# zzuiekongning/MGDT-YOLO

Hardware: AMD Instinct MI355X
Metric: images/sec @640x640 bs=32 per GPU, detection forward + NMS (whole job: 1 GPU(s)) (higher is better)
Workload: dtype bf16; 1 GPU; mspa_c2f_gd_yolov8-n (MSPA-C2f + GD neck + Detect, nc=80) 640x640 inference, batch 32/GPU: forward + decode + NMS(conf 0.25, iou 0.7), hipGraph replay, 4 batches in flight (one captured graph per resident batch, replayed round-robin on 4 streams); global_batch=32, parallelism=replicas x1 (batch-sharded, no data-path collective), rccl_ranks=1, input=bfloat16 NCHW images, 8 different batches resident in HBM (600 MiB) cycled, detections_last_step=9600, weights=seeded random init (no checkpoints offline), batches_in_flight=4

## Files before the change

include/mgdt.h:

```cpp
#ifndef MGDT_H
#define MGDT_H
#include <stddef.h>
#include <stdint.h>

#ifdef __cplusplus
extern "C" {
#endif

typedef void* mgdt_stream;

typedef enum { MGDT_OK = 0, MGDT_BAD_SHAPE = -1, MGDT_BAD_DTYPE = -2, MGDT_LAUNCH_FAIL = -3, MGDT_BAD_ARG = -4,
               MGDT_WORKSPACE = -5 } mgdt_status;
typedef enum { MGDT_F32 = 0, MGDT_BF16 = 1, MGDT_U8 = 2  } mgdt_dtype;
typedef enum { MGDT_ACT_NONE = 0, MGDT_ACT_SILU = 1, MGDT_ACT_RELU = 2, MGDT_ACT_GELU = 3 } mgdt_act;

typedef struct {
  void* p;
  int32_t n, h, w, c;
  int64_t sn, sh, sw, sc;
} mgdt_view;

const char* mgdt_last_error(void);
const char* mgdt_version(void);

size_t mgdt_conv_packed_bytes(int cin, int cout, int k, int dtype);
int mgdt_conv_pack(const float* w_oihw, const float* conv_bias, const float* bn_gamma, const float* bn_beta,
                   const float* bn_mean, const float* bn_var, float bn_eps, int cin, int cout, int k, int dtype,
                   void* packed_out, float* bias_out, mgdt_stream s);
int mgdt_conv_pack_dgrad(const float* w_oihw, int cin, int cout, int k, int phase, int dtype, void* packed_out, float* bias_out, mgdt_stream s);
typedef struct mgdt_pack_desc {
  const float* w; const float* conv_bias; const float* bn_gamma; const float* bn_beta; const float* bn_mean; const float* bn_var;
  float bn_eps; int32_t cin, cout, k, dtype, mode;
  void* packed; float* bias_out;
} mgdt_pack_desc;
int mgdt_conv_pack_batch(const mgdt_pack_desc* descs, int n, mgdt_stream s);

int mgdt_conv2d_fwd(const mgdt_view* x, const mgdt_view* x2, const float* in_scale, const float* in_shift,
                    const void* packed_w, const float* bias, int k, int stride, int act, const mgdt_view* r1,
                    const mgdt_view* r2, const mgdt_view* y, int dtype, mgdt_stream s);
size_t mgdt_conv_packed_bytes_fp8(int cin, int cout, int k);
int mgdt_conv_pack_fp8(const float* w_oihw, const float* conv_bias, const float* bn_gamma, const float* bn_beta, const float* bn_mean,
                       const float* bn_var, float bn_eps, int cin, int cout, int k, float x_qscale, void* packed_out, float* bias_out,
                       float* oscale_out, mgdt_stream s);
int mgdt_conv2d_fp8_fwd(const mgdt_view* x, const mgdt_view* x2, const float* in_scale, const float* in_shift, const void* packed_w,
                        const float* bias, const float* oscale, float x_qscale, int k, int stride, int act, const mgdt_view* r1,
                        const mgdt_view* r2, const mgdt_view* y, mgdt_stream s);
int mgdt_conv2d_phase_fwd(const mgdt_view* x, const void* packed_w, const float* bias, int phase, const mgdt_view* r1, const mgdt_view* r2,
                          const mgdt_view* y, int dtype, mgdt_stream s);

size_t mgdt_cnx_mlp_packed_bytes(int c, int dtype);
int mgdt_cnx_mlp_pack(const float* w1, const float* b1, const float* w2, const float* b2, int c, void* packed, int dtype, mgdt_stream s);
size_t mgdt_cnx_mlp_workspace_bytes(int n, int h, int w, int c);
int mgdt_cnx_mlp_fwd(const mgdt_view* t, const mgdt_view* res, const void* packed, const float* gamma, const float* beta, void* ws,
                     const mgdt_view* y, int dtype, mgdt_stream s);

int mgdt_cnx_block_supported(int n, int h, int w, int c, int dtype);
size_t mgdt_cnx_block_workspace_bytes(int n, int h, int w, int c);
int mgdt_cnx_block_fwd(const mgdt_view* x, const float* dw_w49c, const float* dw_b, const float* ln_w, const float* ln_b, float eps, const void* packed,
                       const float* gamma, const float* beta, const void* tail_w, const float* tail_b, int tail_act, void* ws, size_t ws_bytes,
                       const mgdt_view* y, int dtype, mgdt_stream s);

size_t mgdt_stem2_packed_bytes(void);
int mgdt_stem2_pack(const float* w_folded, void* packed, mgdt_stream s);
int mgdt_stem2_fwd(const mgdt_view* x, int x_dtype, const void* packed0, const float* bias0, const void* packed1, const float* bias1,
                   const mgdt_view* y, mgdt_stream s);
int mgdt_stem2_geometry(int n, int h, int w, int cu_count, int* out);

int mgdt_detect_tail_supported(int c2, int c3, int nc, int reg_max, int dtype);
int mgdt_detect_tail_fwd(const mgdt_view* tb, const mgdt_view* tc, const void* wb, const float* bb, const void* wc, const float* bc, int nc,
                         float stride, int a_off, int a_total, const mgdt_view* feat, float* y, unsigned long long* best_keys,
                         const void* wb3, const float* bb3, mgdt_stream s);
int mgdt_detect_tail_aug_fwd(const mgdt_view* tb, const mgdt_view* tc, const void* wb, const float* bb, const void* wc, const float* bc, int nc,
                             float stride, int a_off, int a_total, const mgdt_view* feat, float* y, unsigned long long* best_keys,
                             const void* wb3, const float* bb3, float aug_scale, int aug_flip, float aug_img_w, mgdt_stream s);

int mgdt_scale_img_fwd(const mgdt_view* x, int x_dtype, int flip, int hs, int ws, float pad, const mgdt_view* y, int y_dtype, mgdt_stream s);

int mgdt_csp_block_supported(int mode, int cin, int cout, int wd, int nbtl, int h, int w, int dtype);
int mgdt_csp_block_tiles(int mode, int n, int cin, int cout, int wd, int nbtl, int h, int w, int* geom8);
int mgdt_csp_block_fwd(int mode, const mgdt_view* x, const void* front, const float* front_bias, const void* const* mid,
                       const float* const* mid_bias, int nbtl, int shortcut, const void* back, const float* back_bias, int wd, int act,
                       const mgdt_view* y, float* pool, int dtype, mgdt_stream s);

size_t mgdt_pw_chain_packed_bytes(int wd, int dtype);
int mgdt_pw_chain_pack(int idx, const float* w_oi, const float* conv_bias, const float* bn_gamma, const float* bn_beta, const float* bn_mean,
                       const float* bn_var, float bn_eps, int wd, int dtype, void* packed, mgdt_stream s);
int mgdt_pw_chain3_fwd(const mgdt_view* x, const void* packed, int wd, int act, const mgdt_view* y, int dtype, mgdt_stream s);

int mgdt_conv1x1_inject_supported(int cin, int cout, int h, int w, int hg, int wg, int dtype);
int mgdt_conv1x1_inject_fwd(const mgdt_view* x, const void* packed_w, const float* bias, const mgdt_view* ga, const mgdt_view* gf,
                            const mgdt_view* y, int dtype, mgdt_stream s);

int mgdt_conv1x1_inject_conv_supported(int cin, int cmid, int cout2, int h, int w, int hg, int wg, int dtype);
int mgdt_conv1x1_inject_conv_fwd(const mgdt_view* x, const void* packed_w, const float* bias, const mgdt_view* ga, const mgdt_view* gf,
                                 const mgdt_view* gsrc, const void* packed_wg, const float* bias_g, int cmid,
                                 const void* packed_w2, const float* bias2, int act2, const mgdt_view* y2, int dtype, mgdt_stream s);

size_t mgdt_groupnorm_workspace_bytes(int n, int c);
int mgdt_groupnorm_fwd(const mgdt_view* x, const float* gamma, const float* beta, int groups, float eps, int act, void* ws, const mgdt_view* y,
                       int dtype, mgdt_stream s);
int mgdt_tood_layer_attn_fwd(const float* sums, int n, int c, int hw, const float* w1, const float* b1, const float* w2, const float* b2, int hid,
                             int stacked, float* scale, mgdt_stream s);
int mgdt_dcnv2_fwd(const mgdt_view* x, const mgdt_view* offset_mask, const float* w_gemm, const float* bias, const mgdt_view* y, int dtype,
                   mgdt_stream s);
int mgdt_dcnv2_mfma_fwd(const mgdt_view* x, const mgdt_view* offset_mask, const void* packed_w, const mgdt_view* y, int dtype, mgdt_stream s);
int mgdt_pixel_gate_fwd(const mgdt_view* x, const mgdt_view* gate, const mgdt_view* y, int dtype, mgdt_stream s);

int mgdt_conv_pack_direct(const float* w_oihw, const float* conv_bias, const float* bn_gamma, const float* bn_beta,
                          const float* bn_mean, const float* bn_var, float bn_eps, int cin_g, int cout, int k,
                          float* w_out, float* bias_out, mgdt_stream s);
int mgdt_conv2d_direct_fwd(const mgdt_view* x, int x_dtype, const float* w_gemm, const float* bias, int k, int stride,
                           int groups, int act, const mgdt_view* y, int dtype, mgdt_stream s);

#define MGDT_SPR_SPLITS 16
int mgdt_spr_pool_fwd(const mgdt_view* x, float* pooled, int dtype, mgdt_stream s);
int mgdt_spr_attn_fwd(const float* pooled, const float* fc1_w, const float* fc1_b, const float* fc2_w,
                      const float* fc2_b, int n, int c, int groups, int h, int w, int softmax, float* attn, mgdt_stream s);
int mgdt_scale_channels_fwd(const mgdt_view* x, const float* attn, const mgdt_view* y, int dtype, mgdt_stream s);
int mgdt_spr_attn_scale_fwd(const float* pooled, int nsplit, int tiles_x, int tiles_y, const float* fc1_w, const float* fc1_b, const float* fc2_w, const float* fc2_b, int groups,
                            const mgdt_view* x, const mgdt_view* y, const mgdt_view* pool_a, const mgdt_view* pool_b, int dtype, mgdt_stream s);

int mgdt_sppf_pool_fwd(const mgdt_view* x, const mgdt_view* y1, const mgdt_view* y2, const mgdt_view* y3, int dtype,
                       mgdt_stream s);

int mgdt_adaptive_avgpool_fwd(const mgdt_view* x, const mgdt_view* y, int dtype, mgdt_stream s);
int mgdt_bilinear_fwd(const mgdt_view* x, const mgdt_view* y, int dtype, mgdt_stream s);
int mgdt_nearest_fwd(const mgdt_view* x, const mgdt_view* y, int dtype, mgdt_stream s);
int mgdt_copy_fwd(const mgdt_view* x, int x_dtype, const mgdt_view* y, int y_dtype, mgdt_stream s);
int mgdt_image_pad4_fwd(const mgdt_view* x, int x_dtype, const mgdt_view* y, int y_dtype, mgdt_stream s);

#define MGDT_GRN_SPLITS 8
int mgdt_dwconv7_ln_fwd(const mgdt_view* x, const float* dw_w, const float* dw_b, const float* ln_w, const float* ln_b,
                        float eps, const mgdt_view* y, int dtype, mgdt_stream s);
int mgdt_grn_stats_fwd(const mgdt_view* t, const float* gamma, float* ws, float* scale, int dtype, mgdt_stream s);

int mgdt_inject_fwd(const mgdt_view* local, const mgdt_view* ga, const mgdt_view* gf, const mgdt_view* y, int dtype,
                    mgdt_stream s);

int mgdt_detect_decode_fwd(const mgdt_view* feat, int reg_max, int nc, float stride, int a_off, int a_total, float* y,
                           int dtype, mgdt_stream s);
int mgdt_detect_decode_aug_fwd(const mgdt_view* feat, int reg_max, int nc, float stride, int a_off, int a_total, float* y,
                               unsigned long long* best_keys, float aug_scale, int aug_flip, float aug_img_w, int dtype, mgdt_stream s);

size_t mgdt_nms_workspace_bytes(int n, int nc, int a, int multi_label, int max_nms);
int mgdt_nms_fwd(const float* pred, int n, int nc, int a, float conf_thres, float iou_thres, const int32_t* classes,
                 int n_classes, int agnostic, int multi_label, int max_det, int max_nms, float max_wh, float* out,
                 int32_t* kept_anchor, int32_t* counts, const unsigned long long* best_keys, void* ws, size_t ws_bytes, mgdt_stream s);

int mgdt_nms_masks_fwd(const float* pred, int n, int nc, int nm, int a, float conf_thres, float iou_thres, const int32_t* classes,
                       int n_classes, int agnostic, int multi_label, int max_det, int max_nms, float max_wh, float* out,
                       int32_t* kept_anchor, int32_t* counts, const unsigned long long* best_keys, void* ws, size_t ws_bytes, mgdt_stream s);

int mgdt_deconv2x2_fwd(const mgdt_view* x, const void* const* packed4, const float* bias, const mgdt_view* y, int dtype, mgdt_stream s);
int mgdt_seg_concat_fwd(const float* y, int n, int rows, int a_total, const mgdt_view* const* mc, int n_levels, int nm, float* out, int dtype,
                        mgdt_stream s);
int mgdt_seg_mask_geometry(int win_h, int win_w, int out_h, int out_w, int* geom4);
int mgdt_seg_masks_fwd(const mgdt_view* protos, const float* rows, const int32_t* counts, const int32_t* offsets, int max_det, int nm,
                       int top, int left, int win_h, int win_w, int out_h, int out_w, int crop_before, float box_sx, float box_sy,
                       int crop_after, int no_skip, void* out, int out_u8, int dtype, mgdt_stream s);

int mgdt_val_match_fwd(const float* det, const int32_t* ndet, int n, int max_det, const float* labels, const int32_t* nlab, int max_lab,
                       const float* iouv, int n_iou, uint8_t* correct, mgdt_stream s);

size_t mgdt_detect_loss_workspace_bytes(int b, int a_total, int n_gt);
int mgdt_detect_loss_fwd(const mgdt_view* const* feats, const float* strides, int n_levels, int reg_max, int nc,
                         const float* gt, int n_gt, int call_count, float gain_box, float gain_cls, float gain_dfl,
                         float* out5, unsigned char* fg_out, int32_t* gt_idx_out, float* tscore_out, void* ws,
                         size_t ws_bytes, int dtype, mgdt_stream s);
int mgdt_detect_loss_fwd_dev(const mgdt_view* const* feats, const float* strides, int n_levels, int reg_max, int nc,
                             const float* gt, int n_gt, const int32_t* call_count_dev, float gain_box, float gain_cls, float gain_dfl,
                             float* out5, unsigned char* fg_out, int32_t* gt_idx_out, float* tscore_out, void* ws,
                             size_t ws_bytes, int dtype, mgdt_stream s);
int mgdt_detect_loss_bwd(const mgdt_view* const* feats, const mgdt_view* const* grads, const float* strides, int n_levels,
                         int reg_max, int nc, const float* gt, int n_gt, float gain_box, float gain_cls, float gain_dfl,
                         float gscale, const float* out5, void* ws, size_t ws_bytes, int dtype, mgdt_stream s);

size_t mgdt_reduce_workspace_bytes(int c);
int mgdt_bn_stats_fwd(const mgdt_view* y, float eps, float momentum, float* mean, float* rstd, float* running_mean,
                      float* running_var, void* ws, int dtype, mgdt_stream s);
int mgdt_bn_act_fwd(const mgdt_view* y, const float* mean, const float* rstd, const float* gamma, const float* beta, int act,
                    const mgdt_view* r1, const mgdt_view* r2, const mgdt_view* z, int dtype, mgdt_stream s);
int mgdt_bn_act_bwd(const mgdt_view* gz, const mgdt_view* y, const float* mean, const float* rstd, const float* gamma,
                    const float* beta, int act, float* dgamma, float* dbeta, const mgdt_view* dy, void* ws, int dtype, mgdt_stream s);
int mgdt_conv_dgrad(const mgdt_view* dy, const float* w_oihw, int k, int stride, const mgdt_view* dx, int accumulate, int dtype,
                    mgdt_stream s);
int mgdt_gconv_dgrad(const mgdt_view* dy, const float* w, int k, int stride, int groups, const mgdt_view* dx, int accumulate, int dtype,
                     mgdt_stream s);
size_t mgdt_gconv_wgrad_workspace_bytes(int cin, int cout, int k, int groups);
int mgdt_gconv_wgrad(const mgdt_view* x, const mgdt_view* dy, int k, int stride, int groups, float* dw, int accumulate, void* ws, int dtype,
                     mgdt_stream s);
size_t mgdt_conv_wgrad_workspace_bytes(int cin, int cout, int k);
int mgdt_conv_wgrad(const mgdt_view* x, const mgdt_view* x2, const mgdt_view* dy, int k, int stride, float* dw_oihw, float* dbias,
                    int accumulate, void* ws, int dtype, mgdt_stream s);
int mgdt_conv_wgrad_splits(int cin, int cout, int k);
typedef struct mgdt_wgrad_final_desc { const float* partial; float* dw; long n; int32_t nsplit; int32_t accumulate; } mgdt_wgrad_final_desc;
int mgdt_wgrad_final_batch(const mgdt_wgrad_final_desc* descs, int n, mgdt_stream s);
int mgdt_add_fwd(const mgdt_view* a, const mgdt_view* b, const mgdt_view* o, int dtype, mgdt_stream s);
int mgdt_maxpool5_bwd(const mgdt_view* x, const mgdt_view* gy, float* gx_f32, int dtype, mgdt_stream s);
int mgdt_nearest_bwd(const mgdt_view* gy, const mgdt_view* gx, int dtype, mgdt_stream s);

int mgdt_ew_binary(const mgdt_view* a, const mgdt_view* b, const mgdt_view* o, int mode, int dtype, mgdt_stream s);
int mgdt_channel_affine(const mgdt_view* x, const float* scale, const float* shift, const mgdt_view* y, int dtype, mgdt_stream s);
size_t mgdt_nc_reduce_workspace_bytes(int n, int c);
int mgdt_nc_reduce(const mgdt_view* a, const mgdt_view* b, float* out, void* ws, int dtype, mgdt_stream s);
int mgdt_adaptive_avgpool_bwd(const mgdt_view* gy, const mgdt_view* gx, int accumulate, int dtype, mgdt_stream s);
int mgdt_bilinear_bwd(const mgdt_view* gy, const mgdt_view* gx, int accumulate, int dtype, mgdt_stream s);
size_t mgdt_spr_bwd_workspace_bytes(int n, int c, int groups);
int mgdt_spr_bwd(const mgdt_view* gy, const float* pooled_partial, int splits, const float* attn, const float* dattn,
                 const float* fc1_w, const float* fc1_b, const float* fc2_w, const float* fc2_b, int groups,
                 const mgdt_view* gx, float* param_grads, void* ws, int dtype, mgdt_stream s);
int mgdt_dwconv7_ln_train_fwd(const mgdt_view* x, const float* dw_w, const float* dw_b, const float* ln_w, const float* ln_b,
                              float eps, const mgdt_view* y, const mgdt_view* u_out, int dtype, mgdt_stream s);
size_t mgdt_dwconv7_ln_bwd_workspace_bytes(int c);
int mgdt_dwconv7_ln_bwd(const mgdt_view* x, const mgdt_view* u, const mgdt_view* gy, const float* dw_w49c, const float* ln_w, float eps,
                        const mgdt_view* du_tmp, const mgdt_view* dx, int accumulate_dx, float* d_dw_w, float* d_dw_b,
                        float* d_ln_w, float* d_ln_b, void* ws, int dtype, mgdt_stream s);
int mgdt_grn_bwd(const mgdt_view* g, const mgdt_view* t, const float* S, const float* A, const float* B, const float* gamma,
                 const mgdt_view* dt, float* dgamma, float* dbeta, void* ws, int dtype, mgdt_stream s);

size_t mgdt_grad_norm_workspace_bytes(void);
int mgdt_grad_clip_coef(const float* g, long n, float max_norm, float* out2, void* ws, mgdt_stream s);
int mgdt_sgd_step(float* p, const float* g, float* buf, const float* wd, long n, float lr, float lr_bias, float momentum, int nesterov,
                  int first, const float* clip2, mgdt_stream s);
int mgdt_ema_update(float* ema, const float* p, long n, float decay, mgdt_stream s);
int mgdt_sgd_ema_step_dev(float* p, const float* g, float* buf, const float* wd, long n_param, float* ema, long n_total, const float* hyper4,
                          int nesterov, int first, const float* clip2, mgdt_stream s);

int mgdt_box_convert(const float* in, float* out, long n, int row, int mode, mgdt_stream s);
int mgdt_box_iou(const float* b1, int n, const float* b2, int m, float eps, float* out, mgdt_stream s);
int mgdt_bbox_iou(const float* b1, int stride1, const float* b2, int stride2, long n, int xywh, int mode, float eps, float* out, mgdt_stream s);
int mgdt_scale_boxes(float* boxes, long n, int row, float gain, float padx, float pady, float h0, float w0, mgdt_stream s);
int mgdt_letterbox_fwd(const void* src_hwc_bgr, int sh, int sw, long src_pitch, void* dst_chw_rgb, int dh, int dw, int new_h, int new_w, int top,
                       int left, mgdt_stream s);
size_t mgdt_ap_workspace_bytes(int n_det, int n_cls);
int mgdt_ap_per_class(const void* tp, const float* conf, const int32_t* seg, const int32_t* nlab, int n_det, int n_cls, int T, const double* x101,
                      const double* px, double eps, void* ws, double* ap, double* pcur, double* rcur, mgdt_stream s);

int mgdt_gn_affine(const float* Sy, const float* Syy, int n, int c, int hw, const float* gamma, const float* beta, int groups, float eps,
                   float* mean_ng, float* rstd_ng, float* A, float* B, mgdt_stream s);
int mgdt_nc_affine_act_bwd(const mgdt_view* g, const mgdt_view* y, const float* A, const float* B, int act, const mgdt_view* gu, int dtype, mgdt_stream s);
size_t mgdt_gn_bwd_workspace_bytes(int n, int c);
int mgdt_gn_bwd_coef(const float* S1, const float* S2, const float* mean_ng, const float* rstd_ng, const float* gamma, int n, int c, int hw, int groups,
                     float* P, float* Q, float* R, float* dgamma, float* dbeta, int accumulate, void* ws, mgdt_stream s);
int mgdt_nc_axpby(const mgdt_view* a, const float* sa, const mgdt_view* b, const float* sb, const float* shift, const mgdt_view* out, int dtype,
                  mgdt_stream s);
int mgdt_pixel_gate_bwd(const mgdt_view* g, const mgdt_view* x, const mgdt_view* logit, const mgdt_view* gx, const mgdt_view* glogit, int dtype, mgdt_stream s);
size_t mgdt_tood_layer_attn_bwd_workspace_bytes(int n, int c, int hid, int stacked);
int mgdt_tood_layer_attn_bwd(const float* sums, const float* dscale, int n, int c, int hw, const float* w1, const float* b1, const float* w2,
                             const float* b2, int hid, int stacked, float* dsums, float* dw1, float* db1, float* dw2, float* db2, int accumulate,
                             void* ws, mgdt_stream s);
int mgdt_dcn_im2col(const mgdt_view* x, const mgdt_view* om, const mgdt_view* col, int dtype, mgdt_stream s);
int mgdt_dcn_col2im_bwd(const mgdt_view* gcol, const mgdt_view* x, const mgdt_view* om, float* gx_f32, const mgdt_view* gom, int dtype, mgdt_stream s);

#ifdef __cplusplus
}
#endif
#endif
```

mgdt_yolo_amd/_lib.py:

```python
import ctypes as C
import os

_HERE = os.path.dirname(os.path.abspath(__file__))
LIB_PATH = os.environ.get('MGDT_LIB') or os.path.join(_HERE, 'csrc', 'libmgdt_hip.so')

F32, BF16 = 0, 1
ACT_NONE, ACT_SILU, ACT_RELU, ACT_GELU = 0, 1, 2, 3
SPR_SPLITS = 16
GRN_SPLITS = 8


class View(C.Structure):
    _fields_ = [('p', C.c_void_p), ('n', C.c_int32), ('h', C.c_int32), ('w', C.c_int32), ('c', C.c_int32),
                ('sn', C.c_int64), ('sh', C.c_int64), ('sw', C.c_int64), ('sc', C.c_int64)]


VP = C.POINTER(View)
_vp, _i, _f, _sz = C.c_void_p, C.c_int, C.c_float, C.c_size_t

class PackDesc(C.Structure):
    _fields_ = [('w', C.c_void_p), ('conv_bias', C.c_void_p), ('bn_gamma', C.c_void_p), ('bn_beta', C.c_void_p), ('bn_mean', C.c_void_p), ('bn_var', C.c_void_p),
                ('bn_eps', C.c_float), ('cin', C.c_int32), ('cout', C.c_int32), ('k', C.c_int32), ('dtype', C.c_int32), ('mode', C.c_int32),
                ('packed', C.c_void_p), ('bias_out', C.c_void_p)]


class WgradFinalDesc(C.Structure):
    _fields_ = [('partial', C.c_void_p), ('dw', C.c_void_p), ('n', C.c_long), ('nsplit', C.c_int32), ('accumulate', C.c_int32)]


PROTOTYPES = {
    'mgdt_last_error': (C.c_char_p, []),
    'mgdt_version': (C.c_char_p, []),
    'mgdt_conv_packed_bytes': (_sz, [_i, _i, _i, _i]),
    'mgdt_conv_pack': (_i, [_vp, _vp, _vp, _vp, _vp, _vp, _f, _i, _i, _i, _i, _vp, _vp, _vp]),
    'mgdt_conv2d_fwd': (_i, [VP, VP, _vp, _vp, _vp, _vp, _i, _i, _i, VP, VP, VP, _i, _vp]),
    'mgdt_conv_packed_bytes_fp8': (_sz, [_i, _i, _i]),
    'mgdt_conv_pack_fp8': (_i, [_vp, _vp, _vp, _vp, _vp, _vp, _f, _i, _i, _i, _f, _vp, _vp, _vp, _vp]),
    'mgdt_conv2d_fp8_fwd': (_i, [VP, VP, _vp, _vp, _vp, _vp, _vp, _f, _i, _i, _i, VP, VP, VP, _vp]),
    'mgdt_conv_pack_batch': (_i, [_vp, _i, _vp]),
    'mgdt_conv2d_phase_fwd': (_i, [VP, _vp, _vp, _i, VP, VP, VP, _i, _vp]),
    'mgdt_conv_wgrad_splits': (_i, [_i, _i, _i]),
    'mgdt_wgrad_final_batch': (_i, [_vp, _i, _vp]),
    'mgdt_conv_pack_dgrad': (_i, [_vp, _i, _i, _i, _i, _i, _vp, _vp, _vp]),
    'mgdt_conv_pack_direct': (_i, [_vp, _vp, _vp, _vp, _vp, _vp, _f, _i, _i, _i, _vp, _vp, _vp]),
    'mgdt_conv2d_direct_fwd': (_i, [VP, _i, _vp, _vp, _i, _i, _i, _i, VP, _i, _vp]),
    'mgdt_spr_pool_fwd': (_i, [VP, _vp, _i, _vp]),
    'mgdt_spr_attn_fwd': (_i, [_vp, _vp, _vp, _vp, _vp, _i, _i, _i, _i, _i, _i, _vp, _vp]),
    'mgdt_scale_channels_fwd': (_i, [VP, _vp, VP, _i, _vp]),
    'mgdt_sppf_pool_fwd': (_i, [VP, VP, VP, VP, _i, _vp]),
    'mgdt_adaptive_avgpool_fwd': (_i, [VP, VP, _i, _vp]),
    'mgdt_bilinear_fwd': (_i, [VP, VP, _i, _vp]),
    'mgdt_nearest_fwd': (_i, [VP, VP, _i, _vp]),
    'mgdt_copy_fwd': (_i, [VP, _i, VP, _i, _vp]),
    'mgdt_image_pad4_fwd': (_i, [VP, _i, VP, _i, _vp]),
    'mgdt_dwconv7_ln_fwd': (_i, [VP, _vp, _vp, _vp, _vp, _f, VP, _i, _vp]),
    'mgdt_cnx_mlp_packed_bytes': (_sz, [_i, _i]),
    'mgdt_cnx_mlp_pack': (_i, [_vp, _vp, _vp, _vp, _i, _vp, _i, _vp]),
    'mgdt_cnx_mlp_workspace_bytes': (_sz, [_i, _i, _i, _i]),
    'mgdt_cnx_mlp_fwd': (_i, [VP, VP, _vp, _vp, _vp, _vp, VP, _i, _vp]),
    'mgdt_cnx_block_supported': (_i, [_i, _i, _i, _i, _i]),
    'mgdt_cnx_block_workspace_bytes': (_sz, [_i, _i, _i, _i]),
    'mgdt_cnx_block_fwd': (_i, [VP, _vp, _vp, _vp, _vp, _f, _vp, _vp, _vp, _vp, _vp, _i, _vp, _sz, VP, _i, _vp]),
    'mgdt_pw_chain_packed_bytes': (_sz, [_i, _i]),
    'mgdt_pw_chain_pack': (_i, [_i, _vp, _vp, _vp, _vp, _vp, _vp, _f, _i, _i, _vp, _vp]),
    'mgdt_pw_chain3_fwd': (_i, [VP, _vp, _i, _i, VP, _i, _vp]),
    'mgdt_conv1x1_inject_supported': (_i, [_i, _i, _i, _i, _i, _i, _i]),
    'mgdt_conv1x1_inject_fwd': (_i, [VP, _vp, _vp, VP, VP, VP, _i, _vp]),
    'mgdt_conv1x1_inject_conv_supported': (_i, [_i, _i, _i, _i, _i, _i, _i, _i]),
    'mgdt_conv1x1_inject_conv_fwd': (_i, [VP, _vp, _vp, VP, VP, VP, _vp, _vp, _i, _vp, _vp, _i, VP, _i, _vp]),
    'mgdt_spr_attn_scale_fwd': (_i, [_vp, _i, _i, _i, _vp, _vp, _vp, _vp, _i, VP, VP, VP, VP, _i, _vp]),
    'mgdt_stem2_packed_bytes': (_sz, []),
    'mgdt_stem2_pack': (_i, [_vp, _vp, _vp]),
    'mgdt_stem2_fwd': (_i, [VP, _i, _vp, _vp, _vp, _vp, VP, _vp]),
    'mgdt_stem2_geometry': (_i, [_i, _i, _i, _i, C.POINTER(C.c_int)]),
    'mgdt_detect_tail_supported': (_i, [_i, _i, _i, _i, _i]),
    'mgdt_detect_tail_fwd': (_i, [VP, VP, _vp, _vp, _vp, _vp, _i, _f, _i, _i, VP, _vp, _vp, _vp, _vp, _vp]),
    'mgdt_detect_tail_aug_fwd': (_i, [VP, VP, _vp, _vp, _vp, _vp, _i, _f, _i, _i, VP, _vp, _vp, _vp, _vp, _f, _i, _f, _vp]),
    'mgdt_scale_img_fwd': (_i, [VP, _i, _i, _i, _i, _f, VP, _i, _vp]),
    'mgdt_csp_block_supported': (_i, [_i, _i, _i, _i, _i, _i, _i, _i]),
    'mgdt_csp_block_tiles': (_i, [_i, _i, _i, _i, _i, _i, _i, _i, _vp]),
    'mgdt_csp_block_fwd': (_i, [_i, VP, _vp, _vp, _vp, _vp, _i, _i, _vp, _vp, _i, _i, VP, _vp, _i, _vp]),
    'mgdt_groupnorm_workspace_bytes': (_sz, [_i, _i]),
    'mgdt_groupnorm_fwd': (_i, [VP, _vp, _vp, _i, _f, _i, _vp, VP, _i, _vp]),
    'mgdt_tood_layer_attn_fwd': (_i, [_vp, _i, _i, _i, _vp, _vp, _vp, _vp, _i, _i, _vp, _vp]),
    'mgdt_dcnv2_fwd': (_i, [VP, VP, _vp, _vp, VP, _i, _vp]),
    'mgdt_dcnv2_mfma_fwd': (_i, [VP, VP, _vp, VP, _i, _vp]),
    'mgdt_pixel_gate_fwd': (_i, [VP, VP, VP, _i, _vp]),
    'mgdt_gn_affine': (_i, [_vp, _vp, _i, _i, _i, _vp, _vp, _i, _f, _vp, _vp, _vp, _vp, _vp]),
    'mgdt_nc_affine_act_bwd': (_i, [VP, VP, _vp, _vp, _i, VP, _i, _vp]),
    'mgdt_gn_bwd_workspace_bytes': (_sz, [_i, _i]),
    'mgdt_gn_bwd_coef': (_i, [_vp, _vp, _vp, _vp, _vp, _i, _i, _i, _i, _vp, _vp, _vp, _vp, _vp, _i, _vp, _vp]),
    'mgdt_nc_axpby': (_i, [VP, _vp, VP, _vp, _vp, VP, _i, _vp]),
    'mgdt_pixel_gate_bwd': (_i, [VP, VP, VP, VP, VP, _i, _vp]),
    'mgdt_tood_layer_attn_bwd_workspace_bytes': (_sz, [_i, _i, _i, _i]),
    'mgdt_tood_layer_attn_bwd': (_i, [_vp, _vp, _i, _i, _i, _vp, _vp, _vp, _vp, _i, _i, _vp, _vp, _vp, _vp, _vp, _i, _vp, _vp]),
    'mgdt_dcn_im2col': (_i, [VP, VP, VP, _i, _vp]),
    'mgdt_dcn_col2im_bwd': (_i, [VP, VP, VP, _vp, VP, _i, _vp]),
    'mgdt_val_match_fwd': (_i, [_vp, _vp, _i, _i, _vp, _vp, _i, _vp, _i, _vp, _vp]),
    'mgdt_grn_stats_fwd': (_i, [VP, _vp, _vp, _vp, _i, _vp]),
    'mgdt_inject_fwd': (_i, [VP, VP, VP, VP, _i, _vp]),
    'mgdt_detect_decode_fwd': (_i, [VP, _i, _i, _f, _i, _i, _vp, _i, _vp]),
    'mgdt_detect_decode_aug_fwd': (_i, [VP, _i, _i, _f, _i, _i, _vp, _vp, _f, _i, _f, _i, _vp]),
    'mgdt_detect_loss_workspace_bytes': (_sz, [_i, _i, _i]),
    'mgdt_detect_loss_fwd': (_i, [_vp, _vp, _i, _i, _i, _vp, _i, _i, _f, _f, _f, _vp, _vp, _vp, _vp, _vp, _sz, _i, _vp]),
    'mgdt_detect_loss_fwd_dev': (_i, [_vp, _vp, _i, _i, _i, _vp, _i, _vp, _f, _f, _f, _vp, _vp, _vp, _vp, _vp, _sz, _i, _vp]),
    'mgdt_detect_loss_bwd': (_i, [_vp, _vp, _vp, _i, _i, _i, _vp, _i, _f, _f, _f, _f, _vp, _vp, _sz, _i, _vp]),
    'mgdt_reduce_workspace_bytes': (_sz, [_i]),
    'mgdt_bn_stats_fwd': (_i, [VP, _f, _f, _vp, _vp, _vp, _vp, _vp, _i, _vp]),
    'mgdt_bn_act_fwd': (_i, [VP, _vp, _vp, _vp, _vp, _i, VP, VP, VP, _i, _vp]),
    'mgdt_bn_act_bwd': (_i, [VP, VP, _vp, _vp, _vp, _vp, _i, _vp, _vp, VP, _vp, _i, _vp]),
    'mgdt_conv_dgrad': (_i, [VP, _vp, _i, _i, VP, _i, _i, _vp]),
    'mgdt_gconv_dgrad': (_i, [VP, _vp, _i, _i, _i, VP, _i, _i, _vp]),
    'mgdt_gconv_wgrad_workspace_bytes': (_sz, [_i, _i, _i, _i]),
    'mgdt_gconv_wgrad': (_i, [VP, VP, _i, _i, _i, _vp, _i, _vp, _i, _vp]),
    'mgdt_conv_wgrad_workspace_bytes': (_sz, [_i, _i, _i]),
    'mgdt_conv_wgrad': (_i, [VP, VP, VP, _i, _i, _vp, _vp, _i, _vp, _i, _vp]),
    'mgdt_add_fwd': (_i, [VP, VP, VP, _i, _vp]),
    'mgdt_maxpool5_bwd': (_i, [VP, VP, _vp, _i, _vp]),
    'mgdt_nearest_bwd': (_i, [VP, VP, _i, _vp]),
    'mgdt_ew_binary': (_i, [VP, VP, VP, _i, _i, _vp]),
    'mgdt_channel_affine': (_i, [VP, _vp, _vp, VP, _i, _vp]),
    'mgdt_nc_reduce_workspace_bytes': (_sz, [_i, _i]),
    'mgdt_nc_reduce': (_i, [VP, VP, _vp, _vp, _i, _vp]),
    'mgdt_adaptive_avgpool_bwd': (_i, [VP, VP, _i, _i, _vp]),
    'mgdt_bilinear_bwd': (_i, [VP, VP, _i, _i, _vp]),
    'mgdt_spr_bwd_workspace_bytes': (_sz, [_i, _i, _i]),
    'mgdt_spr_bwd': (_i, [VP, _vp, _i, _vp, _vp, _vp, _vp, _vp, _vp, _i, VP, _vp, _vp, _i, _vp]),
    'mgdt_dwconv7_ln_train_fwd': (_i, [VP, _vp, _vp, _vp, _vp, _f, VP, VP, _i, _vp]),
    'mgdt_dwconv7_ln_bwd_workspace_bytes': (_sz, [_i]),
    'mgdt_dwconv7_ln_bwd': (_i, [VP, VP, VP, _vp, _vp, _f, VP, VP, _i, _vp, _vp, _vp, _vp, _vp, _i, _vp]),
    'mgdt_grn_bwd': (_i, [VP, VP, _vp, _vp, _vp, _vp, VP, _vp, _vp, _vp, _i, _vp]),
    'mgdt_grad_norm_workspace_bytes': (_sz, []),
    'mgdt_grad_clip_coef': (_i, [_vp, C.c_long, _f, _vp, _vp, _vp]),
    'mgdt_sgd_step': (_i, [_vp, _vp, _vp, _vp, C.c_long, _f, _f, _f, _i, _i, _vp, _vp]),
    'mgdt_ema_update': (_i, [_vp, _vp, C.c_long, _f, _vp]),
    'mgdt_sgd_ema_step_dev': (_i, [_vp, _vp, _vp, _vp, C.c_long, _vp, C.c_long, _vp, _i, _i, _vp, _vp]),
    'mgdt_box_convert': (_i, [_vp, _vp, C.c_long, _i, _i, _vp]),
    'mgdt_box_iou': (_i, [_vp, _i, _vp, _i, _f, _vp, _vp]),
    'mgdt_bbox_iou': (_i, [_vp, _i, _vp, _i, C.c_long, _i, _i, _f, _vp, _vp]),
    'mgdt_scale_boxes': (_i, [_vp, C.c_long, _i, _f, _f, _f, _f, _f, _vp]),
    'mgdt_letterbox_fwd': (_i, [_vp, _i, _i, C.c_long, _vp, _i, _i, _i, _i, _i, _i, _vp]),
    'mgdt_ap_workspace_bytes': (_sz, [_i, _i]),
    'mgdt_ap_per_class': (_i, [_vp, _vp, _vp, _vp, _i, _i, _i, _vp, _vp, C.c_double, _vp, _vp, _vp, _vp, _vp]),
    'mgdt_nms_workspace_bytes': (_sz, [_i, _i, _i, _i, _i]),
    'mgdt_nms_fwd': (_i, [_vp, _i, _i, _i, _f, _f, _vp, _i, _i, _i, _i, _i, _f, _vp, _vp, _vp, _vp, _vp, _sz, _vp]),
    'mgdt_nms_masks_fwd': (_i, [_vp, _i, _i, _i, _i, _f, _f, _vp, _i, _i, _i, _i, _i, _f, _vp, _vp, _vp, _vp, _vp, _sz, _vp]),
    'mgdt_deconv2x2_fwd': (_i, [VP, _vp, _vp, VP, _i, _vp]),
    'mgdt_seg_concat_fwd': (_i, [_vp, _i, _i, _i, _vp, _i, _i, _vp, _i, _vp]),
    'mgdt_seg_mask_geometry': (_i, [_i, _i, _i, _i, C.POINTER(C.c_int)]),
    'mgdt_seg_masks_fwd': (_i, [VP, _vp, _vp, _vp, _i, _i, _i, _i, _i, _i, _i, _i, _i, _f, _f, _i, _i, _vp, _i, _i, _vp]),
}

_lib = None


def lib():
    global _lib
    if _lib is None:
        if not os.path.exists(LIB_PATH):
            raise RuntimeError(f'{LIB_PATH} is missing: build it with `python -c "import __graft_entry__ as g; g.build()"` '
                               '(mgdt_yolo_amd has no CPU or PyTorch fallback)')
        import torch
        l = C.CDLL(LIB_PATH)
        for name, (res, args) in PROTOTYPES.items():
            fn = getattr(l, name)
            fn.restype, fn.argtypes = res, args
        _lib = l
    return _lib


def check(status, what=''):
    if status != 0:
        raise RuntimeError(f'{what or "mgdt"} failed ({status}): {lib().mgdt_last_error().decode()}')
```

mgdt_yolo_amd/csrc/conv3x3_lds.hip:

```cpp
#include <type_traits>
#include <vector>

#include "common.h"

#define C3_OOB ((int)0x80000000)
#define C3_TW 16
#define C3_RW 18
#define C3_MAXI 14

struct C3Args {
  const char* x; int xsn, xsh, xsw; uint32_t x_bytes;
  char* y; int ysn, ysh, ysw; uint32_t y_bytes;
  const char* wpk; const float* bias;
  int N, H, W, Ho, Wo, Cin, Cout, CP, nchunks, NTtot, ncg, tiles_x, tiles_per_img, ntiles, XP, act;
  FastDiv fd_tpi, fd_tx, fd_cp;
  const float* oscale; float xq;
  unsigned long long* dbg;
};

template <int ACT> __device__ __forceinline__ float c3_act(float v) {
  if (ACT == MGDT_ACT_SILU) return v * fast_sigmoid(v);
  if (ACT == MGDT_ACT_RELU) return fmaxf(v, 0.f);
  return v;
}

template <int NBW, int ACT, int NCH, int MT, bool Q8 = false, int S = 1, int WS = 1>
__global__ __launch_bounds__(256 * WS, 1) void conv3x3_lds_kernel(const C3Args a) {
  constexpr int NTHR = 256 * WS, NBH = (NBW + WS - 1) / WS;
  constexpr int RW = 15 * S + 3, TH = 4 * MT, RH = (TH - 1) * S + 3, RPX = RH * RW;
  constexpr int MAXI = ((S == 1 ? C3_MAXI : 18) + WS - 1) / WS;
  constexpr int WB = Q8 ? 512 : 1024, PB = Q8 ? 8 : 16;
  extern __shared__ __attribute__((aligned(16))) char c3_lds[];
  int* tab = (int*)c3_lds;
  char* wl = c3_lds + (((size_t)a.nchunks * 16 + 15) & ~(size_t)15);
  char* xs = wl + (size_t)a.nchunks * NBW * WB;
  const int tid = threadIdx.x, lane = tid & 63, r = lane & 15, g = lane >> 4;
  const int wave_all = __builtin_amdgcn_readfirstlane(tid >> 6);
  const int wave = wave_all & 3, wcol = wave_all >> 2;
  const int cg = blockIdx.x % a.ncg, w0 = blockIdx.x / a.ncg, wstep = gridDim.x / a.ncg;
  const int nb0 = cg * NBW;
  const __amdgpu_buffer_rsrc_t xrs = __builtin_amdgcn_make_buffer_rsrc((void*)a.x, 0, a.x_bytes, 0x00020000);
  const __amdgpu_buffer_rsrc_t yrs = __builtin_amdgcn_make_buffer_rsrc((void*)a.y, 0, a.y_bytes, 0x00020000);

  for (int p = tid; p < a.nchunks * 4; p += NTHR) {
    const int tap = (int)fdiv((uint32_t)p, a.fd_cp), cp = p - tap * a.CP;
    tab[p] = tap < 9 ? ((tap / 3) * RW + (tap % 3)) * a.XP + cp * PB : 0;
  }
  constexpr int WV = WB / 16;
  {
    const int total = a.nchunks * NBW * WV;
    for (int i0 = tid; i0 < total; i0 += 8 * NTHR) {
      uint4 t[8];
#pragma unroll
      for (int u = 0; u < 8; ++u) {
        const int i = min(i0 + u * NTHR, total - 1);
        const int kc = i / (NBW * WV), rem = i - kc * NBW * WV, bw = rem / WV, ln = rem % WV;
        const bool ok = nb0 + bw < a.NTtot;
        t[u] = ok ? *(const uint4*)(a.wpk + ((size_t)(kc * a.NTtot + nb0 + bw) * WV + ln) * 16) : make_uint4(0u, 0u, 0u, 0u);
      }
#pragma unroll
      for (int u = 0; u < 8; ++u)
        if (i0 + u * NTHR < total) *(uint4*)(wl + (size_t)(i0 + u * NTHR) * 16) = t[u];
    }
  }
  const int nbw0 = nb0 + wcol * NBH;
  f32x4 bias[NBH], osc[Q8 ? NBH : 1];
#pragma unroll
  for (int bw = 0; bw < NBH; ++bw) {
    bias[bw] = nbw0 + bw < a.NTtot ? *(const f32x4*)(a.bias + (nbw0 + bw) * 16 + 4 * g) : f32x4{0.f, 0.f, 0.f, 0.f};
    if constexpr (Q8) {
      osc[bw] = nbw0 + bw < a.NTtot ? *(const f32x4*)(a.oscale + (nbw0 + bw) * 16 + 4 * g) : f32x4{1.f, 1.f, 1.f, 1.f};
      bias[bw] = bias[bw] / osc[bw];
    }
  }

  const int nitems = RPX * a.CP;
  uint4 stage[MAXI];
  auto issue = [&](int t) {
    const int n = (int)fdiv((uint32_t)t, a.fd_tpi), rt = t - n * a.tiles_per_img;
    const int tyi = (int)fdiv((uint32_t)rt, a.fd_tx), txi = rt - tyi * a.tiles_x;
    const int iy0 = tyi * TH * S - 1, ix0 = txi * C3_TW * S - 1;
#pragma unroll
    for (int u = 0; u < MAXI; ++u) {
      const int it = tid + u * NTHR;
      const int pix = (int)fdiv((uint32_t)it, a.fd_cp), c8 = it - pix * a.CP;
      const int py = pix / RW, px = pix - py * RW;
      const int iy = iy0 + py, ix = ix0 + px;
      const bool ok = it < nitems && (unsigned)iy < (unsigned)a.H && (unsigned)ix < (unsigned)a.W;
      stage[u] = __builtin_bit_cast(uint4, __builtin_amdgcn_raw_buffer_load_b128(xrs, ok ? (uint32_t)(n * a.xsn + iy * a.xsh + ix * a.xsw + c8 * 16) : (uint32_t)C3_OOB, 0, 0));
    }
  };
  auto commit = [&]() {
#pragma unroll
    for (int u = 0; u < MAXI; ++u) {
      const int it = tid + u * NTHR;
      if (it < nitems) {
        const int pix = (int)fdiv((uint32_t)it, a.fd_cp), c8 = it - pix * a.CP;
        if constexpr (Q8) *(long*)(xs + pix * a.XP + c8 * 8) = quant8(__builtin_bit_cast(bf16x8, stage[u]), a.xq);
        else *(uint4*)(xs + pix * a.XP + c8 * 16) = stage[u];
      }
    }
  };

  const char* const wlane = wl + lane * PB;
  int bbase[MT];
#pragma unroll
  for (int m = 0; m < MT; ++m) bbase[m] = ((wave * MT + m) * S * RW + r * S) * a.XP;

  __builtin_amdgcn_s_waitcnt(0x0F70);
  unsigned long long T0 = 0, Tc = 0, Tm = 0, Te = 0, tl = 0, ntl = 0;
  if (a.dbg) { T0 = __builtin_amdgcn_s_memrealtime(); tl = T0; }
  int t = w0;
  if (t < a.ntiles) issue(t);
  while (t < a.ntiles) {
    __syncthreads();
    commit();
    __syncthreads();
    if (a.dbg) { const unsigned long long n_ = __builtin_amdgcn_s_memrealtime(); Tc += n_ - tl; tl = n_; }
    const int tn = t + wstep;
    if (tn < a.ntiles) issue(tn);

    f32x4 acc[NBH][MT];
#pragma unroll
    for (int bw = 0; bw < NBH; ++bw)
#pragma unroll
      for (int m = 0; m < MT; ++m) acc[bw][m] = bias[bw];
    typedef typename std::conditional<Q8, long, bf16x8>::type frag_t;
    frag_t A[2][NBH], B[2][MT];
    auto load_frags = [&](int kc, int buf) {
      const int off = tab[kc * 4 + g];
#pragma unroll
      for (int bw = 0; bw < NBH; ++bw) A[buf][bw] = *(const frag_t*)(wlane + (size_t)(kc * NBW + wcol * NBH + bw) * WB);
#pragma unroll
      for (int m = 0; m < MT; ++m) B[buf][m] = *(const frag_t*)(xs + bbase[m] + off);
    };
    auto mm = [&](frag_t w, frag_t p, f32x4 c) __attribute__((always_inline)) {
      if constexpr (Q8) return mma_q8(w, p, c);
      else return __builtin_amdgcn_mfma_f32_16x16x32_bf16(w, p, c, 0, 0, 0);
    };
    load_frags(0, 0);
    if (NCH > 0) {
#pragma unroll
      for (int kc = 0; kc < NCH; ++kc) {
        if (kc + 1 < NCH) load_frags(kc + 1, (kc + 1) & 1);
#pragma unroll
        for (int bw = 0; bw < NBH; ++bw)
#pragma unroll
          for (int m = 0; m < MT; ++m) acc[bw][m] = mm(A[kc & 1][bw], B[kc & 1][m], acc[bw][m]);
      }
    } else {
      for (int kc = 0; kc < a.nchunks; kc += 2) {
        if (kc + 1 < a.nchunks) load_frags(kc + 1, 1);
#pragma unroll
        for (int bw = 0; bw < NBH; ++bw)
#pragma unroll
          for (int m = 0; m < MT; ++m) acc[bw][m] = mm(A[0][bw], B[0][m], acc[bw][m]);
        if (kc + 1 < a.nchunks) {
          if (kc + 2 < a.nchunks) load_frags(kc + 2, 0);
#pragma unroll
          for (int bw = 0; bw < NBH; ++bw)
#pragma unroll
            for (int m = 0; m < MT; ++m) acc[bw][m] = mm(A[1][bw], B[1][m], acc[bw][m]);
        }
      }
    }

    if (a.dbg) { const unsigned long long n_ = __builtin_amdgcn_s_memrealtime(); Tm += n_ - tl; tl = n_; }
    {
      const int n = (int)fdiv((uint32_t)t, a.fd_tpi), rt = t - n * a.tiles_per_img;
      const int tyi = (int)fdiv((uint32_t)rt, a.fd_tx), txi = rt - tyi * a.tiles_x;
#pragma unroll
      for (int m = 0; m < MT; ++m) {
        const int oy = tyi * TH + wave * MT + m, ox = txi * C3_TW + r;
        const bool pin = oy < a.Ho && ox < a.Wo;
        const int po = n * a.ysn + oy * a.ysh + ox * a.ysw;
#pragma unroll
        for (int bw = 0; bw < NBH; ++bw) {
          const int co = (nbw0 + bw) * 16 + 4 * g;
          bf16x4 o;
#pragma unroll
          for (int j = 0; j < 4; ++j) o[j] = (bf16)c3_act<ACT>(Q8 ? acc[bw][m][j] * osc[Q8 ? bw : 0][j] : acc[bw][m][j]);
          __builtin_amdgcn_raw_buffer_store_b64(__builtin_bit_cast(__attribute__((__vector_size__(2 * sizeof(unsigned int)))) unsigned int, o), yrs,
                                                (pin && co < a.Cout) ? (uint32_t)(po + co * 2) : (uint32_t)C3_OOB, 0, 0);
        }
      }
    }
    if (a.dbg) { const unsigned long long n_ = __builtin_amdgcn_s_memrealtime(); Te += n_ - tl; tl = n_; ++ntl; }
    t = tn;
  }
  if (a.dbg && tid == 0) { unsigned long long* d = a.dbg + (size_t)blockIdx.x * 6; d[0] = T0; d[1] = tl; d[2] = Tc; d[3] = Tm; d[4] = Te; d[5] = ntl; }
}

bool mgdt_conv3x3_lds_launch(const mgdt_view* x, const mgdt_view* y, const void* packed_w, const float* bias, int act, int CP, int nchunks, int NTtot, hipStream_t st,
                             const float* q8_oscale, float q8_xq, int stride) {
  const bool q8 = q8_oscale != nullptr;
  static const int mode = getenv("MGDT_CONV3_LDS") ? atoi(getenv("MGDT_CONV3_LDS")) : 1;
  if (!mode) return false;
  static const bool ws2 = !(getenv("MGDT_C3_WAVES8") && atoi(getenv("MGDT_C3_WAVES8")) == 0);
  const bool wide = mode >= 3 || ws2;
  const int Cin = x->c, Cout = y->c;
  if (stride == 2 && (q8_oscale || Cin > 64 || NTtot % 4 || (nchunks != 9 && !(nchunks == 18 && wide)))) return false;
  if (Cin % 8 || Cin < 32 || Cin > 80 || Cout % 4 || Cout < 32 || (act != MGDT_ACT_SILU && act != MGDT_ACT_NONE && act != MGDT_ACT_RELU)) return false;
  const long M = (long)x->n * x->h * x->w;
  if (M < 16 * 1024 || x->h < 16 || x->w < 16) return false;
  const long extx = ((long)(x->n - 1) * x->sn + (long)(x->h - 1) * x->sh + (long)(x->w - 1) * x->sw + x->c) * 2;
  const long exty = ((long)(y->n - 1) * y->sn + (long)(y->h - 1) * y->sh + (long)(y->w - 1) * y->sw + y->c) * 2;
  if (extx >= 0x7fffffffL || exty >= 0x7fffffffL) return false;
  C3Args a;
  memset(&a, 0, sizeof(a));
  a.x = (const char*)x->p; a.xsn = (int)(x->sn * 2); a.xsh = (int)(x->sh * 2); a.xsw = (int)(x->sw * 2); a.x_bytes = (uint32_t)extx;
  a.y = (char*)y->p; a.ysn = (int)(y->sn * 2); a.ysh = (int)(y->sh * 2); a.ysw = (int)(y->sw * 2); a.y_bytes = (uint32_t)exty;
  a.wpk = (const char*)packed_w; a.bias = bias;
  a.N = x->n; a.H = x->h; a.W = x->w; a.Ho = y->h; a.Wo = y->w; a.Cin = Cin; a.Cout = Cout; a.CP = CP; a.nchunks = nchunks; a.NTtot = NTtot; a.act = act;
  a.XP = q8 ? Cin + 16 : Cin * 2 + 16;
  a.oscale = q8_oscale; a.xq = q8_xq;
  const int NBW = stride == 2 ? 4 : NTtot;
  if (NBW != 2 && NBW != 3 && NBW != 4 && NBW != 5 && NBW != 6) return false;
  a.ncg = NTtot / NBW;
  const size_t fixed = (((size_t)nchunks * 16 + 15) & ~(size_t)15) + (size_t)nchunks * NBW * (q8 ? 512 : 1024);
  auto region = [&](int mt) { return stride == 2 ? (size_t)(8 * mt + 1) * 33 * a.XP : (size_t)(4 * mt + 2) * C3_RW * a.XP; };
  int MT = stride == 2 ? 2 : 4;
  if (stride == 1 && fixed + region(MT) > 160 * 1024) MT = NBW == 5 && !q8 && wide && fixed + region(3) <= 160 * 1024 ? 3 : 2;
  const size_t lds = fixed + region(MT);
  if (lds > 160 * 1024) return false;
  if (NBW == 5 && !q8 && MT == 2 && mode < 2) return false;
  if (stride == 1 && (q8 ? MT != 4 : ((NBW == 5 && MT == 4) || (NBW != 5 && MT != 4)))) return false;
  const int TH = 4 * MT;
  a.tiles_x = cdiv(y->w, C3_TW);
  a.tiles_per_img = a.tiles_x * cdiv(y->h, TH);
  a.ntiles = x->n * a.tiles_per_img;
  if ((stride == 2 ? (2 * TH + 1) * 33 * CP > 256 * 18 : (TH + 2) * C3_RW * CP > 256 * C3_MAXI)) return false;
  a.fd_tpi = make_fastdiv((uint32_t)a.tiles_per_img); a.fd_tx = make_fastdiv((uint32_t)a.tiles_x); a.fd_cp = make_fastdiv((uint32_t)CP);
  int nwg = 256 / a.ncg * a.ncg;
  nwg = (int)std::min<long>(nwg, (long)a.ntiles * a.ncg);
  nwg = nwg / a.ncg * a.ncg;
  if (nwg < a.ncg) return false;
 #define C3_LAUNCH_Q8(NB, ACTV)                                                                                      \
  {                                                                                                                  \
    static std::atomic<bool> qattr{false}, qattr18{false}, qattr23{false};                                            \
    if (nchunks == 18) {                                                                                             \
      if (!qattr18) { (void)hipFuncSetAttribute((const void*)conv3x3_lds_kernel<NB, ACTV, 18, 4, true>, hipFuncAttributeMaxDynamicSharedMemorySize, 160 * 1024); qattr18 = true; } \
      conv3x3_lds_kernel<NB, ACTV, 18, 4, true><<<nwg, 256, lds, st>>>(a);                                           \
    } else if (nchunks == 23) {                                                                                      \
      if (!qattr23) { (void)hipFuncSetAttribute((const void*)conv3x3_lds_kernel<NB, ACTV, 23, 4, true>, hipFuncAttributeMaxDynamicSharedMemorySize, 160 * 1024); qattr23 = true; } \
      conv3x3_lds_kernel<NB, ACTV, 23, 4, true><<<nwg, 256, lds, st>>>(a);                                           \
    } else {                                                                                                         \
      if (!qattr) { (void)hipFuncSetAttribute((const void*)conv3x3_lds_kernel<NB, ACTV, 0, 4, true>, hipFuncAttributeMaxDynamicSharedMemorySize, 160 * 1024); qattr = true; } \
      conv3x3_lds_kernel<NB, ACTV, 0, 4, true><<<nwg, 256, lds, st>>>(a);                                            \
    }                                                                                                                \
  }
#define C3_ACT_Q8(NB) \
  if (act == MGDT_ACT_SILU) C3_LAUNCH_Q8(NB, MGDT_ACT_SILU) else if (act == MGDT_ACT_RELU) C3_LAUNCH_Q8(NB, MGDT_ACT_RELU) else C3_LAUNCH_Q8(NB, MGDT_ACT_NONE)
#define C3_LAUNCH(NB, ACTV, MTV, WSV)                                                                                     \
  {                                                                                                                  \
    static std::atomic<bool> attr{false}, attr18{false}, attr23{false};                                                                        \
    if (nchunks == 18) {                                                                                             \
      if (!attr18) { (void)hipFuncSetAttribute((const void*)conv3x3_lds_kernel<NB, ACTV, 18, MTV, false, 1, WSV>, hipFuncAttributeMaxDynamicSharedMemorySize, 160 * 1024); attr18 = true; } \
      conv3x3_lds_kernel<NB, ACTV, 18, MTV, false, 1, WSV><<<nwg, 256 * WSV, lds, st>>>(a);                                                    \
    } else if (nchunks == 23) {                                                                                      \
      if (!attr23) { (void)hipFuncSetAttribute((const void*)conv3x3_lds_kernel<NB, ACTV, 23, MTV, false, 1, WSV>, hipFuncAttributeMaxDynamicSharedMemorySize, 160 * 1024); attr23 = true; } \
      conv3x3_lds_kernel<NB, ACTV, 23, MTV, false, 1, WSV><<<nwg, 256 * WSV, lds, st>>>(a);                                               \
    } else {                                                                                                         \
      if (!attr) { (void)hipFuncSetAttribute((const void*)conv3x3_lds_kernel<NB, ACTV, 0, MTV, false, 1, WSV>, hipFuncAttributeMaxDynamicSharedMemorySize, 160 * 1024); attr = true; } \
      conv3x3_lds_kernel<NB, ACTV, 0, MTV, false, 1, WSV><<<nwg, 256 * WSV, lds, st>>>(a);                                                     \
    }                                                                                                                \
  }
#define C3_ACT(NB, MTV, WSV) \
  if (act == MGDT_ACT_SILU) C3_LAUNCH(NB, MGDT_ACT_SILU, MTV, WSV) else if (act == MGDT_ACT_RELU) C3_LAUNCH(NB, MGDT_ACT_RELU, MTV, WSV) else C3_LAUNCH(NB, MGDT_ACT_NONE, MTV, WSV)
  static unsigned long long* dbgbuf = nullptr;
  if (getenv("MGDT_C3_DBG") && !dbgbuf) (void)hipMalloc((void**)&dbgbuf, 256 * 6 * 8);
  a.dbg = dbgbuf;
#define C3_LAUNCH_S2(ACTV, NCHV)                                                                                      \
  {                                                                                                                  \
    static std::atomic<bool> sattr{false}, sattr8{false};                                                            \
    if (ws2) {                                                                                                       \
      if (!sattr8) { (void)hipFuncSetAttribute((const void*)conv3x3_lds_kernel<4, ACTV, NCHV, 2, false, 2, 2>, hipFuncAttributeMaxDynamicSharedMemorySize, 160 * 1024); sattr8 = true; } \
      conv3x3_lds_kernel<4, ACTV, NCHV, 2, false, 2, 2><<<nwg, 512, lds, st>>>(a);                                   \
    } else {                                                                                                         \
      if (!sattr) { (void)hipFuncSetAttribute((const void*)conv3x3_lds_kernel<4, ACTV, NCHV, 2, false, 2>, hipFuncAttributeMaxDynamicSharedMemorySize, 160 * 1024); sattr = true; } \
      conv3x3_lds_kernel<4, ACTV, NCHV, 2, false, 2><<<nwg, 256, lds, st>>>(a);                                      \
    }                                                                                                                \
  }
#define C3_ACT_S2(NCHV) \
  if (act == MGDT_ACT_SILU) C3_LAUNCH_S2(MGDT_ACT_SILU, NCHV) else if (act == MGDT_ACT_RELU) C3_LAUNCH_S2(MGDT_ACT_RELU, NCHV) else C3_LAUNCH_S2(MGDT_ACT_NONE, NCHV)
  if (stride == 2) {
    if (nchunks == 9) { C3_ACT_S2(9) } else { C3_ACT_S2(18) }
  } else if (q8) {
    if (NBW == 6) { C3_ACT_Q8(6) } else if (NBW == 5) { C3_ACT_Q8(5) } else if (NBW == 4) { C3_ACT_Q8(4) } else if (NBW == 3) { C3_ACT_Q8(3) } else { C3_ACT_Q8(2) }
  } else if (ws2 && (NBW == 6 || NBW == 4 || (NBW == 5 && MT == 3))) {
    if (NBW == 6) { C3_ACT(6, 4, 2) } else if (NBW == 4) { C3_ACT(4, 4, 2) } else { C3_ACT(5, 3, 2) }
  } else if (NBW == 6) { C3_ACT(6, 4, 1) } else if (NBW == 5 && MT == 3) { C3_ACT(5, 3, 1) } else if (NBW == 5) { C3_ACT(5, 2, 1) } else if (NBW == 4) { C3_ACT(4, 4, 1) } else if (NBW == 3) { C3_ACT(3, 4, 1) } else { C3_ACT(2, 4, 1) }
#undef C3_ACT
#undef C3_ACT_Q8
#undef C3_ACT_S2
#undef C3_LAUNCH_S2
#undef C3_LAUNCH_Q8
#undef C3_LAUNCH
  if (dbgbuf) {
    std::vector<unsigned long long> h(256 * 6);
    (void)hipStreamSynchronize(st);
    (void)hipMemcpy(h.data(), dbgbuf, h.size() * 8, hipMemcpyDeviceToHost);
    unsigned long long t0 = ~0ull, t1 = 0; double c = 0, m = 0, e = 0, nt = 0;
    for (int i = 0; i < nwg; ++i) { t0 = std::min(t0, h[i * 6]); t1 = std::max(t1, h[i * 6 + 1]); c += h[i * 6 + 2]; m += h[i * 6 + 3]; e += h[i * 6 + 4]; nt += h[i * 6 + 5]; }
    fprintf(stderr, "conv3x3_lds cin %d cout %d %dx%d: %d wgs, %d tiles, span %.1f us; per tile (us): wait+commit %.2f mfma %.2f epilogue %.2f\n", Cin, Cout, x->h, x->w, nwg,
            a.ntiles, (t1 - t0) * 0.01, c / nt * 0.01, m / nt * 0.01, e / nt * 0.01);
  }
  return true;
}
```

mgdt_yolo_amd/csrc/conv_igemm.hip:

```cpp
#include "conv_igemm_kernel.h"

struct FoldArgs { const float *cb, *g, *b, *mu, *var; float eps; int cout_real, cpad; float* bias_out; };
template <typename T>
__global__ void pack_kernel(const float* __restrict__ w, const float* __restrict__ scale, int Cin, int Cout, int KS,
                            int CP, int nchunks, int NTtot, T* __restrict__ out, int dgrad = 0, FoldArgs fa = FoldArgs{}) {
  constexpr int PE = Piece<T>::PE;
  long total = (long)nchunks * NTtot * 64 * PE;
  if (fa.bias_out && blockIdx.x == 0)
    for (int c = threadIdx.x; c < fa.cpad; c += blockDim.x) {
      float bo = 0.f;
      if (c < fa.cout_real) {
        if (fa.g) {
          const float s = fa.g[c] / sqrtf(fa.eps + fa.var[c]);
          bo = fa.b[c] - fa.g[c] * fa.mu[c] / sqrtf(fa.var[c] + fa.eps);
          if (fa.cb) bo += s * fa.cb[c];
        } else if (fa.cb) {
          bo = fa.cb[c];
        }
      }
      fa.bias_out[c] = bo;
    }
  for (long i = blockIdx.x * (long)blockDim.x + threadIdx.x; i < total; i += (long)gridDim.x * blockDim.x) {
    int j = (int)(i % PE);
    long t = i / PE;
    int lane = (int)(t % 64);
    t /= 64;
    int nb = (int)(t % NTtot);
    int kc = (int)(t / NTtot);
    int r = lane & 15, g = lane >> 4;
    int p = kc * 4 + g;
    int tap = p / CP, cp = p % CP;
    if (dgrad >= 2) {
      const int nc_ = 1 + ((dgrad - 2) & 1), nr_ = 1 + ((dgrad - 2) >> 1);
      tap = tap < nr_ * nc_ ? (1 + tap / nc_) * 3 + (1 + tap % nc_) : 99;
    }
    int cin = cp * PE + j, cout = nb * 16 + r;
    float v = 0.f;
    if (tap < KS * KS && cin < Cin && cout < Cout) {
      if (dgrad == 1) v = w[(((long)cin * Cout + cout) * KS + (KS - 1 - tap / KS)) * KS + (KS - 1 - tap % KS)];
      else if (dgrad >= 2) {
        const int py = (dgrad - 2) >> 1, px = (dgrad - 2) & 1;
        const int ky = py + 1 - 2 * (tap / KS - 1), kx = px + 1 - 2 * (tap % KS - 1);
        v = ((unsigned)ky < 3u && (unsigned)kx < 3u) ? w[(((long)cin * Cout + cout) * 3 + ky) * 3 + kx] : 0.f;
      }
      else v = w[(((long)cout * Cin + cin) * KS + tap / KS) * KS + tap % KS];
      if (scale) v *= scale[cout];
      else if (fa.g) v *= fa.g[cout] / sqrtf(fa.eps + fa.var[cout]);
    }
    out[i] = (T)v;
  }
}

__global__ void fold_kernel(const float* cb, const float* g, const float* b, const float* mu, const float* var, float eps,
                            int Cout, int Cpad, float* scale, float* bias_out) {
  int c = blockIdx.x * blockDim.x + threadIdx.x;
  if (c >= Cpad) return;
  float s = 1.f, bo = 0.f;
  if (c < Cout) {
    if (g) {
      s = g[c] / sqrtf(eps + var[c]);
      bo = b[c] - g[c] * mu[c] / sqrtf(var[c] + eps);
      if (cb) bo += s * cb[c];
    } else if (cb) {
      bo = cb[c];
    }
  }
  scale[c] = s;
  bias_out[c] = bo;
}

static inline int piece_elems(int dtype) { return dtype == MGDT_BF16 ? 8 : 4; }

static inline int phase_ntaps(int mode) { return mode < 2 ? 9 : (1 + ((mode - 2) >> 1)) * (1 + ((mode - 2) & 1)); }
static inline unsigned long long phase_taplist(int mode, int k) {
  unsigned long long l = 0;
  if (mode < 2) { for (int t = 0; t < k * k; ++t) l |= (unsigned long long)t << (4 * t); return l; }
  const int nr = 1 + ((mode - 2) >> 1), nc = 1 + ((mode - 2) & 1);
  for (int i = 0; i < nr * nc; ++i) l |= (unsigned long long)((1 + i / nc) * 3 + (1 + i % nc)) << (4 * i);
  return l;
}
static void conv_geometry(int cin, int cout, int k, int dtype, int* CP, int* nchunks, int* NTtot, int ntaps = 0) {
  int pe = piece_elems(dtype);
  *CP = (cin + pe - 1) / pe;
  int pieces = (ntaps > 0 ? ntaps : k * k) * (*CP);
  *nchunks = (pieces + 3) / 4;
  *NTtot = (cout + 15) / 16;
}

extern "C" size_t mgdt_conv_packed_bytes(int cin, int cout, int k, int dtype) {
  int CP, nchunks, NTtot;
  conv_geometry(cin, cout, k, dtype, &CP, &nchunks, &NTtot);
  return (size_t)nchunks * NTtot * 1024 + (size_t)NTtot * 16 * sizeof(float);
}

extern "C" int mgdt_conv_pack(const float* w, const float* cb, const float* g, const float* b, const float* mu,
                              const float* var, float eps, int cin, int cout, int k, int dtype, void* packed,
                              float* bias_out, mgdt_stream s) {
  if (!w || !packed || !bias_out) MGDT_FAIL(MGDT_BAD_ARG, "conv_pack: null pointer");
  if ((g != nullptr) != (b != nullptr) || (g != nullptr) != (mu != nullptr) || (g != nullptr) != (var != nullptr))
    MGDT_FAIL(MGDT_BAD_ARG, "conv_pack: BN arguments must be all present or all NULL");
  int CP, nchunks, NTtot;
  conv_geometry(cin, cout, k, dtype, &CP, &nchunks, &NTtot);
  hipStream_t st = (hipStream_t)s;
  float* scale = (float*)((char*)packed + (size_t)nchunks * NTtot * 1024);
  int cpad = NTtot * 16;
  (void)scale;
  long total = (long)nchunks * NTtot * 64 * piece_elems(dtype);
  int grid = (int)std::min<long>((total + 255) / 256, 4096);
  const FoldArgs fa{cb, g, b, mu, var, eps, cout, cpad, bias_out};
  MGDT_DISPATCH_DTYPE(dtype, (pack_kernel<T><<<grid, 256, 0, st>>>(w, nullptr, cin, cout, k, CP, nchunks, NTtot, (T*)packed, 0, fa)));
  MGDT_CHECK_LAUNCH("conv_pack");
  return MGDT_OK;
}

extern "C" int mgdt_conv_pack_dgrad(const float* w, int cin, int cout, int k, int phase, int dtype, void* packed, float* bias_out, mgdt_stream s) {
  if (!w || !packed || !bias_out) MGDT_FAIL(MGDT_BAD_ARG, "conv_pack_dgrad: null pointer");
  if (phase < -1 || phase > 3 || (phase >= 0 && k != 3)) MGDT_FAIL(MGDT_BAD_SHAPE, "conv_pack_dgrad: phase %d (stride-2 phases need k = 3)", phase);
  int CP, nchunks, NTtot;
  conv_geometry(cout, cin, k, dtype, &CP, &nchunks, &NTtot, phase < 0 ? 0 : phase_ntaps(2 + phase));
  hipStream_t st = (hipStream_t)s;
  float* scale = (float*)((char*)packed + (size_t)nchunks * NTtot * 1024);
  const int cpad = NTtot * 16;
  (void)scale;
  long total = (long)nchunks * NTtot * 64 * piece_elems(dtype);
  int grid = (int)std::min<long>((total + 255) / 256, 4096);
  const FoldArgs fa{nullptr, nullptr, nullptr, nullptr, nullptr, 0.f, cin, cpad, bias_out};
  MGDT_DISPATCH_DTYPE(dtype, (pack_kernel<T><<<grid, 256, 0, st>>>(w, nullptr, cout, cin, k, CP, nchunks, NTtot, (T*)packed, phase < 0 ? 1 : 2 + phase, fa)));
  MGDT_CHECK_LAUNCH("conv_pack_dgrad");
  return MGDT_OK;
}

__global__ void q8_wscale_kernel(const float* __restrict__ w, FoldArgs fa, int per_cout, float xq, float* __restrict__ wscale, float* __restrict__ oscale) {
  const int c = blockIdx.x;
  __shared__ float red[256];
  float m = 0.f;
  if (c < fa.cout_real)
    for (int i = threadIdx.x; i < per_cout; i += blockDim.x) m = fmaxf(m, fabsf(w[(long)c * per_cout + i]));
  red[threadIdx.x] = m;
  __syncthreads();
  for (int s = 128; s > 0; s >>= 1) {
    if ((int)threadIdx.x < s) red[threadIdx.x] = fmaxf(red[threadIdx.x], red[threadIdx.x + s]);
    __syncthreads();
  }
  if (threadIdx.x == 0) {
    float bo = 0.f, ws = 1.f;
    if (c < fa.cout_real) {
      float fold = 1.f;
      if (fa.g) {
        fold = fa.g[c] / sqrtf(fa.eps + fa.var[c]);
        bo = fa.b[c] - fa.g[c] * fa.mu[c] / sqrtf(fa.var[c] + fa.eps);
        if (fa.cb) bo += fold * fa.cb[c];
      } else if (fa.cb) {
        bo = fa.cb[c];
      }
      const float amax = red[0] * fabsf(fold);
      ws = amax > 0.f ? amax / 448.f : 1.f;
    }
    wscale[c] = ws;
    oscale[c] = ws / xq;
    fa.bias_out[c] = bo;
  }
}
__global__ void pack_q8_kernel(const float* __restrict__ w, FoldArgs fa, const float* __restrict__ wscale, int Cin, int Cout, int KS, int CP, int nchunks,
                               int NTtot, long* __restrict__ out) {
  typedef __attribute__((ext_vector_type(2))) int i32x2;
  const long total = (long)nchunks * NTtot * 64;
  for (long t = blockIdx.x * (long)blockDim.x + threadIdx.x; t < total; t += (long)gridDim.x * blockDim.x) {
    const int lane = (int)(t % 64);
    const int nb = (int)((t / 64) % NTtot), kc = (int)(t / 64 / NTtot);
    const int r = lane & 15, g = lane >> 4;
    const int p = kc * 4 + g, tap = p / CP, cp = p % CP, cout = nb * 16 + r;
    float v[8];
#pragma unroll
    for (int j = 0; j < 8; ++j) {
      const int cin = cp * 8 + j;
      float q = 0.f;
      if (tap < KS * KS && cin < Cin && cout < Cout) {
        q = w[(((long)cout * Cin + cin) * KS + tap / KS) * KS + tap % KS];
        if (fa.g) q *= fa.g[cout] / sqrtf(fa.eps + fa.var[cout]);
        q = __builtin_amdgcn_fmed3f(q / wscale[cout], -448.f, 448.f);
      }
      v[j] = q;
    }
    i32x2 o = {0, 0};
    o[0] = __builtin_amdgcn_cvt_pk_fp8_f32(v[0], v[1], o[0], false);
    o[0] = __builtin_amdgcn_cvt_pk_fp8_f32(v[2], v[3], o[0], true);
    o[1] = __builtin_amdgcn_cvt_pk_fp8_f32(v[4], v[5], o[1], false);
    o[1] = __builtin_amdgcn_cvt_pk_fp8_f32(v[6], v[7], o[1], true);
    out[t] = __builtin_bit_cast(long, o);
  }
}

extern "C" size_t mgdt_conv_packed_bytes_fp8(int cin, int cout, int k) {
  int CP, nchunks, NTtot;
  conv_geometry(cin, cout, k, MGDT_BF16, &CP, &nchunks, &NTtot);
  return (size_t)nchunks * NTtot * 512 + (size_t)NTtot * 16 * sizeof(float);
}

extern "C" int mgdt_conv_pack_fp8(const float* w, const float* cb, const float* g, const float* b, const float* mu, const float* var, float eps,
                                  int cin, int cout, int k, float x_qscale, void* packed, float* bias_out, float* oscale_out, mgdt_stream s) {
  if (!w || !packed || !bias_out || !oscale_out) MGDT_FAIL(MGDT_BAD_ARG, "conv_pack_fp8: null pointer");
  if ((g != nullptr) != (b != nullptr) || (g != nullptr) != (mu != nullptr) || (g != nullptr) != (var != nullptr))
    MGDT_FAIL(MGDT_BAD_ARG, "conv_pack_fp8: BN arguments must be all present or all NULL");
  if (!(x_qscale > 0.f) || !(x_qscale < 3.0e38f)) MGDT_FAIL(MGDT_BAD_ARG, "conv_pack_fp8: x_qscale must be a positive finite number");
  if (cin % 8 || cout % 4 || (k != 1 && k != 3)) MGDT_FAIL(MGDT_BAD_SHAPE, "conv_pack_fp8: cin=%d must be a multiple of 8, cout=%d of 4, k=%d 1 or 3", cin, cout, k);
  int CP, nchunks, NTtot;
  conv_geometry(cin, cout, k, MGDT_BF16, &CP, &nchunks, &NTtot);
  hipStream_t st = (hipStream_t)s;
  float* wscale = (float*)((char*)packed + (size_t)nchunks * NTtot * 512);
  const int cpad = NTtot * 16;
  const FoldArgs fa{cb, g, b, mu, var, eps, cout, cpad, bias_out};
  q8_wscale_kernel<<<cpad, 256, 0, st>>>(w, fa, cin * k * k, x_qscale, wscale, oscale_out);
  const long total = (long)nchunks * NTtot * 64;
  pack_q8_kernel<<<(int)std::min<long>((total + 255) / 256, 4096), 256, 0, st>>>(w, fa, wscale, cin, cout, k, CP, nchunks, NTtot, (long*)packed);
  MGDT_CHECK_LAUNCH("conv_pack_fp8");
  return MGDT_OK;
}

struct PackJob { const float* w; FoldArgs fa; int Cin, Cout, KS, CP, nchunks, NTtot, dgrad; void* out; };
#define PACK_BATCH 16
struct PackJobs { PackJob j[PACK_BATCH]; };
template <typename T>
__global__ void pack_batch_kernel(const PackJobs jobs) {
  const PackJob& J = jobs.j[blockIdx.y];
  constexpr int PE = Piece<T>::PE;
  const long total = (long)J.nchunks * J.NTtot * 64 * PE;
  const FoldArgs fa = J.fa;
  if (fa.bias_out && blockIdx.x == 0)
    for (int c = threadIdx.x; c < fa.cpad; c += blockDim.x) {
      float bo = 0.f;
      if (c < fa.cout_real) {
        if (fa.g) {
          const float s = fa.g[c] / sqrtf(fa.eps + fa.var[c]);
          bo = fa.b[c] - fa.g[c] * fa.mu[c] / sqrtf(fa.var[c] + fa.eps);
          if (fa.cb) bo += s * fa.cb[c];
        } else if (fa.cb) {
          bo = fa.cb[c];
        }
      }
      fa.bias_out[c] = bo;
    }
  const int Cin = J.Cin, Cout = J.Cout, KS = J.KS, CP = J.CP, NTtot = J.NTtot, dgrad = J.dgrad;
  const float* __restrict__ w = J.w;
  T* __restrict__ out = (T*)J.out;
  for (long i = blockIdx.x * (long)blockDim.x + threadIdx.x; i < total; i += (long)gridDim.x * blockDim.x) {
    int j = (int)(i % PE);
    long t = i / PE;
    int lane = (int)(t % 64);
    t /= 64;
    int nb = (int)(t % NTtot);
    int kc = (int)(t / NTtot);
    int r = lane & 15, g = lane >> 4;
    int p = kc * 4 + g;
    int tap = p / CP, cp = p % CP;
    if (dgrad >= 2) {
      const int nc_ = 1 + ((dgrad - 2) & 1), nr_ = 1 + ((dgrad - 2) >> 1);
      tap = tap < nr_ * nc_ ? (1 + tap / nc_) * 3 + (1 + tap % nc_) : 99;
    }
    int cin = cp * PE + j, cout = nb * 16 + r;
    float v = 0.f;
    if (tap < KS * KS && cin < Cin && cout < Cout) {
      if (dgrad == 1) v = w[(((long)cin * Cout + cout) * KS + (KS - 1 - tap / KS)) * KS + (KS - 1 - tap % KS)];
      else if (dgrad >= 2) {
        const int py = (dgrad - 2) >> 1, px = (dgrad - 2) & 1;
        const int ky = py + 1 - 2 * (tap / KS - 1), kx = px + 1 - 2 * (tap % KS - 1);
        v = ((unsigned)ky < 3u && (unsigned)kx < 3u) ? w[(((long)cin * Cout + cout) * 3 + ky) * 3 + kx] : 0.f;
      }
      else v = w[(((long)cout * Cin + cin) * KS + tap / KS) * KS + tap % KS];
      if (fa.g) v *= fa.g[cout] / sqrtf(fa.eps + fa.var[cout]);
    }
    out[i] = (T)v;
  }
}

extern "C" int mgdt_conv_pack_batch(const mgdt_pack_desc* d, int n, mgdt_stream s) {
  if (!d || n < 0) MGDT_FAIL(MGDT_BAD_ARG, "conv_pack_batch: null descriptor array");
  hipStream_t st = (hipStream_t)s;
  for (int dtype : {MGDT_F32, MGDT_BF16}) {
    PackJobs jobs;
    int m = 0;
    auto flush = [&]() {
      if (!m) return;
      for (int q = m; q < PACK_BATCH; ++q) { jobs.j[q] = jobs.j[0]; jobs.j[q].nchunks = 0; jobs.j[q].fa.bias_out = nullptr; }
      if (dtype == MGDT_F32) pack_batch_kernel<float><<<dim3(32, m), 256, 0, st>>>(jobs);
      else pack_batch_kernel<bf16><<<dim3(32, m), 256, 0, st>>>(jobs);
      m = 0;
    };
    for (int i = 0; i < n; ++i) {
      const mgdt_pack_desc& e = d[i];
      if (e.dtype != dtype) continue;
      if (!e.w || !e.packed || !e.bias_out) MGDT_FAIL(MGDT_BAD_ARG, "conv_pack_batch: descriptor %d has a null pointer", i);
      if (e.mode < 0 || e.mode > 5 || (e.mode >= 2 && e.k != 3)) MGDT_FAIL(MGDT_BAD_SHAPE, "conv_pack_batch: descriptor %d mode %d", i, e.mode);
      PackJob& J = jobs.j[m++];
      const int gi = e.mode == 0 ? e.cin : e.cout, go = e.mode == 0 ? e.cout : e.cin;
      conv_geometry(gi, go, e.k, dtype, &J.CP, &J.nchunks, &J.NTtot, e.mode >= 2 ? phase_ntaps(e.mode) : 0);
      J.w = e.w; J.Cin = gi; J.Cout = go; J.KS = e.k; J.dgrad = e.mode; J.out = e.packed;
      J.fa = e.mode == 0 ? FoldArgs{e.conv_bias, e.bn_gamma, e.bn_beta, e.bn_mean, e.bn_var, e.bn_eps, go, J.NTtot * 16, e.bias_out}
                         : FoldArgs{nullptr, nullptr, nullptr, nullptr, nullptr, 0.f, go, J.NTtot * 16, e.bias_out};
      if (m == PACK_BATCH) flush();
    }
    flush();
  }
  MGDT_CHECK_LAUNCH("conv_pack_batch");
  return MGDT_OK;
}

bool mgdt_conv3x3_lds_launch(const mgdt_view* x, const mgdt_view* y, const void* packed_w, const float* bias, int act, int CP, int nchunks, int NTtot, hipStream_t st,
                             const float* q8_oscale, float q8_xq, int stride);

template <typename T, int NT, int MT, bool Q8>
int launch_igemm(const ConvArgs& a, int gx, int gy, int threads, size_t lds, hipStream_t st);

template <typename T>
static int dispatch_igemm(const ConvArgs& a, int NT, int MT, int gx, int gy, int threads, size_t lds, hipStream_t st) {
#define CASE(nt, mt) \
  if (NT == nt && MT == mt) return launch_igemm<T, nt, mt, false>(a, gx, gy, threads, lds, st);
  CASE(1, 2) CASE(1, 4) CASE(2, 2) CASE(3, 2) CASE(4, 2) CASE(5, 2) CASE(6, 2) CASE(8, 2)
#undef CASE
  MGDT_FAIL(MGDT_BAD_SHAPE, "conv2d: no kernel for NT=%d MT=%d", NT, MT);
}

static int dispatch_igemm_q8(const ConvArgs& a, int NT, int gx, int gy, int threads, size_t lds, hipStream_t st) {
#define CASE(nt) \
  if (NT == nt) return launch_igemm<bf16, nt, 2, true>(a, gx, gy, threads, lds, st);
  CASE(1) CASE(2) CASE(3) CASE(4) CASE(5) CASE(6) CASE(8)
#undef CASE
  MGDT_FAIL(MGDT_BAD_SHAPE, "conv2d_fp8: no kernel for NT=%d", NT);
}

static int conv2d_fwd_impl(const mgdt_view* x, const mgdt_view* x2, const float* in_scale, const float* in_shift,
                           const void* packed_w, const float* bias, int k, int stride, int act, const mgdt_view* r1,
                           const mgdt_view* r2, const mgdt_view* y, int dtype, int tapmode, mgdt_stream s,
                           const float* q8_oscale = nullptr, float q8_xq = 1.f);
extern "C" int mgdt_conv2d_fwd(const mgdt_view* x, const mgdt_view* x2, const float* in_scale, const float* in_shift,
                               const void* packed_w, const float* bias, int k, int stride, int act, const mgdt_view* r1,
                               const mgdt_view* r2, const mgdt_view* y, int dtype, mgdt_stream s) {
  return conv2d_fwd_impl(x, x2, in_scale, in_shift, packed_w, bias, k, stride, act, r1, r2, y, dtype, 0, s);
}
extern "C" int mgdt_conv2d_phase_fwd(const mgdt_view* x, const void* packed_w, const float* bias, int phase, const mgdt_view* r1, const mgdt_view* r2,
                                     const mgdt_view* y, int dtype, mgdt_stream s) {
  if (phase < 0 || phase > 3) MGDT_FAIL(MGDT_BAD_ARG, "conv2d_phase: phase %d", phase);
  return conv2d_fwd_impl(x, nullptr, nullptr, nullptr, packed_w, bias, 3, 1, MGDT_ACT_NONE, r1, r2, y, dtype, 2 + phase, s);
}
extern "C" int mgdt_conv2d_fp8_fwd(const mgdt_view* x, const mgdt_view* x2, const float* in_scale, const float* in_shift,
                                   const void* packed_w, const float* bias, const float* oscale, float x_qscale, int k, int stride, int act,
                                   const mgdt_view* r1, const mgdt_view* r2, const mgdt_view* y, mgdt_stream s) {
  if (!oscale) MGDT_FAIL(MGDT_BAD_ARG, "conv2d_fp8: null oscale");
  if (!(x_qscale > 0.f) || !(x_qscale < 3.0e38f)) MGDT_FAIL(MGDT_BAD_ARG, "conv2d_fp8: x_qscale must be a positive finite number");
  return conv2d_fwd_impl(x, x2, in_scale, in_shift, packed_w, bias, k, stride, act, r1, r2, y, MGDT_BF16, 0, s, oscale, x_qscale);
}
static int conv2d_fwd_impl(const mgdt_view* x, const mgdt_view* x2, const float* in_scale, const float* in_shift,
                           const void* packed_w, const float* bias, int k, int stride, int act, const mgdt_view* r1,
                           const mgdt_view* r2, const mgdt_view* y, int dtype, int tapmode, mgdt_stream s,
                           const float* q8_oscale, float q8_xq) {
  const bool q8 = q8_oscale != nullptr;
  const int WB = q8 ? 512 : 1024;
  if (!view_ok(x) || !view_ok(y) || !packed_w || !bias) MGDT_FAIL(MGDT_BAD_ARG, "conv2d: null/empty view or weights");
  if (dtype != MGDT_F32 && dtype != MGDT_BF16) MGDT_FAIL(MGDT_BAD_DTYPE, "conv2d: dtype %d", dtype);
  if ((k != 1 && k != 3) || (stride != 1 && stride != 2)) MGDT_FAIL(MGDT_BAD_SHAPE, "conv2d: k=%d stride=%d unsupported", k, stride);
  const int pe = piece_elems(dtype);
  const int pad = k / 2;
  const int Ho = (x->h + 2 * pad - k) / stride + 1, Wo = (x->w + 2 * pad - k) / stride + 1;
  if (y->n != x->n || y->h != Ho || y->w != Wo) MGDT_FAIL(MGDT_BAD_SHAPE, "conv2d: y is %dx%dx%d, expected %dx%dx%d", y->n, y->h, y->w, x->n, Ho, Wo);
  if (x->c % pe || y->c % 4) MGDT_FAIL(MGDT_BAD_SHAPE, "conv2d: cin=%d must be a multiple of %d and cout=%d of 4", x->c, pe, y->c);
  auto aligned = [&](const mgdt_view* v, int q) {
    return v->sc == 1 && v->sw % q == 0 && v->sh % q == 0 && v->sn % q == 0 && ((uintptr_t)v->p % (q * dtype_size(dtype))) == 0;
  };
  if (!aligned(x, pe) || !aligned(y, 4)) MGDT_FAIL(MGDT_BAD_SHAPE, "conv2d: x/y must be NHWC views (sc==1) with 16-byte aligned pieces");
  if (x2 && x2->p && (x2->n != x->n || x2->h != x->h || x2->w != x->w || x2->c != x->c || !aligned(x2, pe)))
    MGDT_FAIL(MGDT_BAD_SHAPE, "conv2d: x2 must match x");
  for (const mgdt_view* rr : {r1, r2})
    if (rr && rr->p && (rr->n != y->n || rr->h != Ho || rr->w != Wo || rr->c != y->c || !aligned(rr, 4)))
      MGDT_FAIL(MGDT_BAD_SHAPE, "conv2d: residual must match y");

  ConvArgs a;
  memset(&a, 0, sizeof(a));
  const long sz = (long)dtype_size(dtype);
  auto extent = [&](const mgdt_view* v) { return ((long)(v->n - 1) * v->sn + (long)(v->h - 1) * v->sh + (long)(v->w - 1) * v->sw + v->c) * sz; };
  bool fits = true;
  auto bind = [&](const mgdt_view* v, const char** p, int* sn, int* sh, int* sw, uint32_t* bytes) {
    if (!v || !v->p) return;
    if (extent(v) >= 0x7fffffffL || v->sh * sz >= (1L << 23) || v->sw * sz >= (1L << 23)) { fits = false; return; }
    *p = (const char*)v->p; *sn = (int)(v->sn * sz); *sh = (int)(v->sh * sz); *sw = (int)(v->sw * sz); *bytes = (uint32_t)extent(v);
  };
  const char* yp = nullptr;
  bind(x, &a.x, &a.xsn, &a.xsh, &a.xsw, &a.x_bytes);
  bind(x2, &a.x2, &a.x2sn, &a.x2sh, &a.x2sw, &a.x2_bytes);
  bind(y, &yp, &a.ysn, &a.ysh, &a.ysw, &a.y_bytes);
  bind(r1, &a.r1, &a.r1sn, &a.r1sh, &a.r1sw, &a.r1_bytes);
  bind(r2, &a.r2, &a.r2sn, &a.r2sh, &a.r2sw, &a.r2_bytes);
  if (!fits) MGDT_FAIL(MGDT_BAD_SHAPE, "conv2d: a view spans >= 2 GiB or has a row stride >= 8 MiB");
  a.y = (char*)yp;
  a.in_scale = in_scale; a.in_shift = in_shift;
  a.wpk = (const char*)packed_w; a.bias = bias;
  a.oscale = q8_oscale; a.xq = q8_xq;
  a.N = x->n; a.H = x->h; a.W = x->w; a.Cin = x->c; a.Ho = Ho; a.Wo = Wo; a.Cout = y->c;
  a.KS = k; a.stride = stride; a.pad = pad; a.act = act;
  a.ntaps = tapmode >= 2 ? phase_ntaps(tapmode) : k * k;
  a.taplist = phase_taplist(tapmode, k);
  conv_geometry(a.Cin, a.Cout, k, dtype, &a.CP, &a.nchunks, &a.NTtot, tapmode >= 2 ? a.ntaps : 0);
  long M = (long)a.N * Ho * Wo;
  if (M > 0x7fffffffL - (1 << 20)) MGDT_FAIL(MGDT_BAD_SHAPE, "conv2d: problem too large");
  a.M = (int)M; a.HoWo = Ho * Wo;
  a.fd_howo = make_fastdiv((uint32_t)a.HoWo); a.fd_wo = make_fastdiv((uint32_t)Wo);
  if (tapmode == 0 && dtype == MGDT_BF16 && k == 3 && !(x2 && x2->p) && !in_scale && !in_shift && !(r1 && r1->p) && !(r2 && r2->p) &&
      mgdt_conv3x3_lds_launch(x, y, packed_w, bias, act, a.CP, a.nchunks, a.NTtot, (hipStream_t)s, q8_oscale, q8_xq, stride)) {
    MGDT_CHECK_LAUNCH("conv2d(3x3 lds)");
    return MGDT_OK;
  }

  int LDS_PANEL_KIB = 144;
  { const char* e = getenv("MGDT_CONV_PANEL_KIB"); if (e) LDS_PANEL_KIB = atoi(e); }
  int NT = 1;
  for (int c : {8, 6, 5, 4, 3, 2, 1})
    if (a.NTtot % c == 0 && (long)a.nchunks * c * WB <= LDS_PANEL_KIB * 1024L) { NT = c; break; }
  int MT = 2;
  if (!q8 && NT == 1 && a.NTtot == 1) { const char* e = getenv("MGDT_CONV_MT1"); MT = e && atoi(e) == 4 ? 4 : 2; }
  int waves = 8;
  auto wgs = [&](int nt, int wv) { return (long)cdiv(M, 16 * wv * MT) * (a.NTtot / nt); };
  {
    const char* e = getenv("MGDT_CONV_MINWG");
    const int minwg = e ? atoi(e) : 128;
    while (wgs(NT, waves) < minwg && NT > 1 && NT % 2 == 0) NT /= 2;
  }
  {
    static const bool tail_split = getenv("MGDT_CONV_TAIL_SPLIT") != nullptr;
    const long w0 = wgs(NT, waves);
    if (tail_split && w0 > 768 && w0 <= 960 && NT % 2 == 0) NT /= 2;
  }
  {
    const char* e;
    if ((e = getenv("MGDT_CONV_WAVES"))) waves = std::min(8, std::max(1, atoi(e)));
  }
  a.numTiles = cdiv(M, 16 * waves * MT);
  a.T8 = cdiv(a.numTiles, 8);
  a.tab_bytes = (a.nchunks + 3) / 4 * 4 * 4 * 16;
  size_t panel = (size_t)a.nchunks * NT * WB;
  if (panel <= (size_t)LDS_PANEL_KIB * 1024) { a.seg_chunks = a.nchunks; a.nseg = 1; }
  else { a.seg_chunks = 64; a.nseg = cdiv(a.nchunks, a.seg_chunks); }
  size_t lds = a.tab_bytes + (size_t)(q8 ? 2 : 1) * NT * 16 * sizeof(float) + (size_t)a.seg_chunks * NT * WB;
  int gcap = waves == 8 ? 256 : 1024;
  { const char* e = getenv("MGDT_CONV_GCAP"); if (e) gcap = atoi(e); }
  if (lds > 160 * 1024) MGDT_FAIL(MGDT_BAD_SHAPE, "conv2d: %zu bytes of LDS for NT=%d, %d chunks", lds, NT, a.seg_chunks);
  int gx = std::min(8 * a.T8, gcap), gy = a.NTtot / NT;
  hipStream_t st = (hipStream_t)s;
  if (q8) return dispatch_igemm_q8(a, NT, gx, gy, waves * 64, lds, st);
  if (dtype == MGDT_F32) return dispatch_igemm<float>(a, NT, MT, gx, gy, waves * 64, lds, st);
  return dispatch_igemm<bf16>(a, NT, MT, gx, gy, waves * 64, lds, st);
}
```

mgdt_yolo_amd/csrc/detect_tail.hip:

```cpp
#include "conv_igemm_kernel.h"

struct DtArgs {
  const char* tb; int bsn, bsh, bsw; uint32_t tb_bytes;
  const char* tc; int csn, csh, csw; uint32_t tc_bytes;
  char* feat; int fsn, fsh, fsw; uint32_t feat_bytes;
  const char* wb; const float* bb; const char* wc; const float* bc;
  float* y;
  unsigned long long* best;
  const char* wb3; const float* bb3;
  int N, H, W, HW, c2, c3, nc, kch, nbc, units_per_img, units, a_off, a_total;
  float stride;
  FastDiv fd_w;
  int aug, aug_flip;
  float aug_s, aug_w;
};

constexpr int DT_THREADS = 256;
constexpr int DT_P = 20;
constexpr int DT_WT = (2 * 16 + 4) * DT_P;

__global__ __launch_bounds__(DT_THREADS) void detect_tail_kernel(const DtArgs a) {
  extern __shared__ __attribute__((aligned(16))) char smem[];
  char* wbl = smem;
  char* wcl = smem + 1024;
  float* biasl = (float*)(wcl + (size_t)a.kch * a.nbc * 1024);
  float* ytile = biasl + 16 + a.nbc * 16;
  char* wb3l = (char*)(ytile + (size_t)4 * DT_WT);
  float* bias3l = (float*)(wb3l + 5 * 1024);
  const int tid = threadIdx.x, lane = tid & 63;
  const int wave = __builtin_amdgcn_readfirstlane(tid >> 6);
  const int r = lane & 15, g = lane >> 4;
  for (int i = tid; i < 64; i += DT_THREADS) ((uint4*)wbl)[i] = ((const uint4*)a.wb)[i];
  for (int i = tid; i < a.kch * a.nbc * 64; i += DT_THREADS) ((uint4*)wcl)[i] = ((const uint4*)a.wc)[i];
  for (int i = tid; i < 16 + a.nbc * 16; i += DT_THREADS) biasl[i] = i < 16 ? a.bb[i] : a.bc[i - 16];
  if (a.wb3) {
    for (int i = tid; i < 5 * 64; i += DT_THREADS) ((uint4*)wb3l)[i] = ((const uint4*)a.wb3)[i];
    if (tid < 16) bias3l[tid] = a.bb3[tid];
  }
  __syncthreads();
  const __amdgpu_buffer_rsrc_t brs = __builtin_amdgcn_make_buffer_rsrc((void*)a.tb, 0, a.tb_bytes, 0x00020000);
  const __amdgpu_buffer_rsrc_t crs = __builtin_amdgcn_make_buffer_rsrc((void*)a.tc, 0, a.tc_bytes, 0x00020000);
  const __amdgpu_buffer_rsrc_t frs = __builtin_amdgcn_make_buffer_rsrc((void*)a.feat, 0, a.feat_bytes, 0x00020000);
  float* yt = ytile + (size_t)wave * DT_WT;
  const char* wlane_b = wbl + lane * 16;
  const char* wlane_c = wcl + lane * 16;
  const int boff = (8 * g < a.c2) ? g * 16 : MGDT_OOB;
  const int r4 = 16;

  const bool vec_ok = (a.HW & 3) == 0 && (a.a_off & 3) == 0 && (a.a_total & 3) == 0 && ((uintptr_t)a.y & 15) == 0;
  auto wave_sync = [&]() __attribute__((always_inline)) {
    __builtin_amdgcn_fence(__ATOMIC_RELEASE, "wavefront");
    __builtin_amdgcn_wave_barrier();
    __builtin_amdgcn_fence(__ATOMIC_ACQUIRE, "wavefront");
  };
  auto flush = [&](const float* tile, int nrow, int row0, int n, int an0) __attribute__((always_inline)) {
    const int row = lane >> 2, q = (lane & 3) * 4;
    if (row < nrow && row0 + row < 4 + a.nc) {
      float* dst = a.y + ((size_t)n * (4 + a.nc) + row0 + row) * a.a_total + a.a_off + an0 + q;
      const float* src = tile + row * DT_P + q;
      if (vec_ok) { if (an0 + q < a.HW) *(f32x4*)dst = *(const f32x4*)src; }
      else {
#pragma unroll
        for (int e = 0; e < 4; ++e) if (an0 + q + e < a.HW) dst[e] = src[e];
      }
    }
  };
  int flip = 0;
  for (int unit = blockIdx.x * 4 + wave; unit < a.units; unit += gridDim.x * 4) {
    const int n = unit / a.units_per_img, a0 = (unit - n * a.units_per_img) * 32;
    float bs[2] = {-1.f, -1.f};
    int bcl[2] = {0, 0};
#pragma unroll
    for (int u = 0; u < 2; ++u) {
      const int an = a0 + u * 16 + r;
      const bool pv = an < a.HW;
      const int oy = (int)fdiv((uint32_t)(pv ? an : 0), a.fd_w), ox = (pv ? an : 0) - oy * a.W;
      const int bo = pv ? n * a.bsn + oy * a.bsh + ox * a.bsw : MGDT_OOB;
      const int co = pv ? n * a.csn + oy * a.csh + ox * a.csw : MGDT_OOB;
      const int fo = pv ? n * a.fsn + oy * a.fsh + ox * a.fsw : MGDT_OOB;
      bf16x8 Bb;
      if (a.wb3) {
        bf16x8 B3[5];
#pragma unroll
        for (int kc = 0; kc < 5; ++kc) {
          const int p = kc * 4 + g, tap = p >> 1, cp = p & 1;
          const int iy = oy + tap / 3 - 1, ix = ox + tap % 3 - 1;
          const bool ok = pv && tap < 9 && (unsigned)iy < (unsigned)a.H && (unsigned)ix < (unsigned)a.W;
          B3[kc] = __builtin_bit_cast(bf16x8, __builtin_amdgcn_raw_buffer_load_b128(brs, ok ? (uint32_t)(n * a.bsn + iy * a.bsh + ix * a.bsw + cp * 16) : (uint32_t)MGDT_OOB, 0, 0));
        }
        f32x4 acc3 = *(const f32x4*)(bias3l + 4 * g);
#pragma unroll
        for (int kc = 0; kc < 5; ++kc) acc3 = mma(*(const bf16x8*)(wb3l + kc * 1024 + lane * 16), B3[kc], acc3);
#pragma unroll
        for (int e = 0; e < 8; ++e) Bb[e] = e < 4 ? (bf16)(acc3[e] * fast_sigmoid(acc3[e])) : (bf16)0.f;
      } else {
        Bb = __builtin_bit_cast(bf16x8, __builtin_amdgcn_raw_buffer_load_b128(brs, (bo | boff) < 0 ? (uint32_t)MGDT_OOB : (uint32_t)(bo + boff), 0, 0));
      }
      bf16x8 Bc[4];
#pragma unroll
      for (int kc = 0; kc < 4; ++kc) {
        const int piece = kc * 4 + g;
        const bool ok = kc < a.kch && piece * 8 < a.c3;
        Bc[kc] = __builtin_bit_cast(bf16x8, __builtin_amdgcn_raw_buffer_load_b128(crs, (ok && co >= 0) ? (uint32_t)(co + piece * 16) : (uint32_t)MGDT_OOB, 0, 0));
      }
      f32x4 accb = *(const f32x4*)(biasl + 4 * g);
      accb = mma(*(const bf16x8*)wlane_b, Bb, accb);
      float lb[4];
#pragma unroll
      for (int j = 0; j < 4; ++j) lb[j] = (float)(bf16)accb[j];
      bstore4<bf16>(frs, (uint32_t)fo + (uint32_t)(4 * g * 2), f32x4{lb[0], lb[1], lb[2], lb[3]});
      const float mx = fmaxf(fmaxf(lb[0], lb[1]), fmaxf(lb[2], lb[3]));
      float den = 0.f, num = 0.f;
#pragma unroll
      for (int k = 0; k < 4; ++k) {
        const float e = __builtin_amdgcn_exp2f((lb[k] - mx) * 1.4426950408889634f);
        den += e;
        num += e * (float)k;
      }
      const float dd = num * __builtin_amdgcn_rcpf(den);
      const float dl = __shfl(dd, r, 64), dt = __shfl(dd, 16 + r, 64), dr = __shfl(dd, 32 + r, 64), db = __shfl(dd, 48 + r, 64);
      const float ax = (float)ox + 0.5f, ay = (float)oy + 0.5f;
      const float x1 = ax - dl, y1 = ay - dt, x2 = ax + dr, y2 = ay + db;
      float comp = g == 0 ? (x1 + x2) / 2.f * a.stride : g == 1 ? (y1 + y2) / 2.f * a.stride : g == 2 ? (x2 - x1) * a.stride : (y2 - y1) * a.stride;
      if (a.aug) {
        comp = comp / a.aug_s;
        if (g == 0 && a.aug_flip) comp = a.aug_w - comp;
      }
      {
        float* bt = yt + 32 * DT_P;
        bt[g * DT_P + r] = comp;
        wave_sync();
        flush(bt, 4, 0, n, a0 + u * 16);
      }
      for (int nb = 0; nb < a.nbc; ++nb) {
        f32x4 acc = *(const f32x4*)(biasl + 16 + nb * 16 + 4 * g);
#pragma unroll
        for (int kc = 0; kc < 4; ++kc)
          if (kc < a.kch) acc = mma(*(const bf16x8*)(wlane_c + (size_t)(kc * a.nbc + nb) * 1024), Bc[kc], acc);
        const int c = nb * 16 + 4 * g;
        float lc[4];
#pragma unroll
        for (int j = 0; j < 4; ++j) lc[j] = (float)(bf16)acc[j];
        bstore4<bf16>(frs, c < a.nc ? (uint32_t)fo + (uint32_t)((r4 + c) * 2) : (uint32_t)MGDT_OOB, f32x4{lc[0], lc[1], lc[2], lc[3]});
        float* ct = yt + flip * 16 * DT_P;
        flip ^= 1;
#pragma unroll
        for (int j = 0; j < 4; ++j) {
          const float sg = fast_sigmoid(lc[j]);
          ct[(4 * g + j) * DT_P + r] = sg;
          if (c + j < a.nc && sg > bs[u]) { bs[u] = sg; bcl[u] = c + j; }
        }
        wave_sync();
        flush(ct, 16, 4 + nb * 16, n, a0 + u * 16);
      }
    }
    if (a.best) {
#pragma unroll
      for (int u = 0; u < 2; ++u) {
#pragma unroll
        for (int off = 16; off <= 32; off <<= 1) {
          const float os = __shfl_xor(bs[u], off, 64);
          const int oc = __shfl_xor(bcl[u], off, 64);
          if (os > bs[u] || (os == bs[u] && oc < bcl[u])) { bs[u] = os; bcl[u] = oc; }
        }
        if (g == 0 && a0 + u * 16 + r < a.HW) {
          const unsigned an = (unsigned)(a.a_off + a0 + u * 16 + r);
          a.best[(size_t)n * a.a_total + an] = ((unsigned long long)(0xFFFFFFFFu - __float_as_uint(bs[u])) << 32) | (unsigned long long)(an * (unsigned)a.nc + (unsigned)bcl[u]);
        }
      }
    }
    wave_sync();
  }
}

extern "C" int mgdt_detect_tail_supported(int c2, int c3, int nc, int reg_max, int dtype) {
  return dtype == MGDT_BF16 && reg_max == 4 && c2 % 8 == 0 && c2 <= 32 && c3 % 8 == 0 && c3 <= 128 && nc >= 4 && nc <= 256 && nc % 4 == 0;
}

static int detect_tail_launch(const mgdt_view* tb, const mgdt_view* tc, const void* wb, const float* bb, const void* wc, const float* bc, int nc,
                              float stride, int a_off, int a_total, const mgdt_view* feat, float* y, unsigned long long* best_keys,
                              const void* wb3, const float* bb3, bool aug, float aug_scale, int aug_flip, float aug_img_w, mgdt_stream s) {
  if (!view_ok(tb) || !view_ok(tc) || !view_ok(feat) || !wb || !bb || !wc || !bc || !y) MGDT_FAIL(MGDT_BAD_ARG, "detect_tail: null/empty argument");
  if (!mgdt_detect_tail_supported(tb->c, tc->c, nc, 4, MGDT_BF16)) MGDT_FAIL(MGDT_BAD_SHAPE, "detect_tail: c2=%d c3=%d nc=%d not covered", tb->c, tc->c, nc);
  if (feat->c != 16 + nc || tb->n != tc->n || tb->h != tc->h || tb->w != tc->w || feat->n != tb->n || feat->h != tb->h || feat->w != tb->w ||
      a_off < 0 || a_off + tb->h * tb->w > a_total)
    MGDT_FAIL(MGDT_BAD_SHAPE, "detect_tail: shapes");
  DtArgs a;
  memset(&a, 0, sizeof(a));
  bool fits = true;
  auto bind = [&](const mgdt_view* v, const char** p, int* sn, int* sh, int* sw, uint32_t* bytes, int q) {
    const long ext = ((long)(v->n - 1) * v->sn + (long)(v->h - 1) * v->sh + (long)(v->w - 1) * v->sw + v->c) * 2;
    if (v->sc != 1 || v->sw % q || v->sh % q || v->sn % q || (uintptr_t)v->p % (q * 2) || ext >= 0x7fffffffL) { fits = false; return; }
    *p = (const char*)v->p; *sn = (int)(v->sn * 2); *sh = (int)(v->sh * 2); *sw = (int)(v->sw * 2); *bytes = (uint32_t)ext;
  };
  const char* fp = nullptr;
  bind(tb, &a.tb, &a.bsn, &a.bsh, &a.bsw, &a.tb_bytes, 8);
  bind(tc, &a.tc, &a.csn, &a.csh, &a.csw, &a.tc_bytes, 8);
  bind(feat, &fp, &a.fsn, &a.fsh, &a.fsw, &a.feat_bytes, 4);
  if (!fits) MGDT_FAIL(MGDT_BAD_SHAPE, "detect_tail: views must be 16-byte aligned NHWC (sc == 1) below 2 GiB");
  a.feat = (char*)fp;
  a.wb = (const char*)wb; a.bb = bb; a.wc = (const char*)wc; a.bc = bc; a.y = y; a.best = best_keys;
  a.wb3 = (const char*)wb3; a.bb3 = bb3;
  if (wb3 && (!bb3 || tb->c != 16)) MGDT_FAIL(MGDT_BAD_SHAPE, "detect_tail: the in-launch 3x3 box conv is built for 16 -> 16 channels");
  a.N = tb->n; a.H = tb->h; a.W = tb->w; a.HW = tb->h * tb->w; a.c2 = tb->c; a.c3 = tc->c; a.nc = nc;
  a.kch = cdiv(tc->c, 32); a.nbc = cdiv(nc, 16);
  a.units_per_img = cdiv(a.HW, 32); a.units = a.N * a.units_per_img;
  a.a_off = a_off; a.a_total = a_total; a.stride = stride; a.fd_w = make_fastdiv((uint32_t)tb->w);
  a.aug = aug ? 1 : 0; a.aug_flip = aug_flip ? 1 : 0; a.aug_s = aug_scale; a.aug_w = aug_img_w;
  const size_t lds = 1024 + (size_t)a.kch * a.nbc * 1024 + (size_t)(16 + a.nbc * 16) * 4 + (size_t)4 * DT_WT * 4 + 5 * 1024 + 64;
  if (lds > 150 * 1024) MGDT_FAIL(MGDT_BAD_SHAPE, "detect_tail: nc=%d needs %zu B of LDS", nc, lds);
  static size_t attr = 0;
  if (lds > 64 * 1024 && lds > attr) {
    hipError_t e = hipFuncSetAttribute((const void*)detect_tail_kernel, hipFuncAttributeMaxDynamicSharedMemorySize, 150 * 1024);
    if (e != hipSuccess) MGDT_FAIL(MGDT_LAUNCH_FAIL, "detect_tail: hipFuncSetAttribute: %s", hipGetErrorString(e));
    attr = 150 * 1024;
  }
  const int grid = std::min(cdiv(a.units, 4), 1024);
  detect_tail_kernel<<<grid, DT_THREADS, lds, (hipStream_t)s>>>(a);
  MGDT_CHECK_LAUNCH("detect_tail_fwd");
  return MGDT_OK;
}

extern "C" int mgdt_detect_tail_fwd(const mgdt_view* tb, const mgdt_view* tc, const void* wb, const float* bb, const void* wc, const float* bc, int nc,
                                    float stride, int a_off, int a_total, const mgdt_view* feat, float* y, unsigned long long* best_keys,
                                    const void* wb3, const float* bb3, mgdt_stream s) {
  return detect_tail_launch(tb, tc, wb, bb, wc, bc, nc, stride, a_off, a_total, feat, y, best_keys, wb3, bb3, false, 1.f, 0, 0.f, s);
}

extern "C" int mgdt_detect_tail_aug_fwd(const mgdt_view* tb, const mgdt_view* tc, const void* wb, const float* bb, const void* wc, const float* bc, int nc,
                                        float stride, int a_off, int a_total, const mgdt_view* feat, float* y, unsigned long long* best_keys,
                                        const void* wb3, const float* bb3, float aug_scale, int aug_flip, float aug_img_w, mgdt_stream s) {
  if (!(aug_scale > 0.f)) MGDT_FAIL(MGDT_BAD_ARG, "detect_tail_aug: scale %g", (double)aug_scale);
  return detect_tail_launch(tb, tc, wb, bb, wc, bc, nc, stride, a_off, a_total, feat, y, best_keys, wb3, bb3, true, aug_scale, aug_flip, aug_img_w, s);
}
```

mgdt_yolo_amd/nn/modules/head.py:

```python
import math

import torch
import torch.nn as nn

from ... import ops
from .block import DFL, Proto
from .conv import Conv, HipModule

__all__ = ('Detect', 'Segment', 'TOODHead', 'Conv_GN', 'TaskDecomposition', 'DyDCNv2', 'Scale')


class _HeadConv(HipModule):

    @staticmethod
    def run(owner, conv, x, out):
        q = 4
        mfma = (conv.out_channels % q == 0 and out.stride(3) % q == 0 and out.stride(2) % q == 0 and out.stride(0) % q == 0 and
                out.data_ptr() % (q * out.element_size()) == 0 and
                ops.conv_can_mfma(x, conv.in_channels, conv.out_channels, 1, 1, 1, out.dtype))
        pk = owner._cached((id(conv), out.dtype, mfma), [conv.weight, conv.bias],
                           lambda: ops.PackedConv(conv.weight, conv.bias, None, 1, out.dtype, direct=not mfma))
        return ops.conv2d(x, pk, 1, ops.ACT_NONE, out=out)

    @staticmethod
    def backward(conv, x, g, accumulate=False):
        ops.grad_buf(conv.weight)
        ops.grad_buf(conv.bias)
        ops.conv_wgrad(x, g, 1, 1, conv.weight.grad, dbias=conv.bias.grad, accumulate=accumulate)
        dx = ops.new_act(x.shape[0], x.shape[1], x.shape[2], x.shape[3], x.dtype, x.device)
        return ops.conv_dgrad(g, conv.weight, 1, 1, dx)


class Detect(HipModule):
    dynamic = False
    export = False
    shape = None
    anchors = torch.empty(0)
    strides = torch.empty(0)

    def __init__(self, nc=80, ch=()):
        super().__init__()
        self.nc = nc
        self.nl = len(ch)
        self.reg_max = 4
        self.no = nc + self.reg_max * 4
        self.stride = torch.zeros(self.nl)
        c2, c3 = max((16, ch[0] // 4, self.reg_max * 4)), max(ch[0], self.nc)
        self.cv2 = nn.ModuleList(nn.Sequential(Conv(x, c2, 3), Conv(c2, c2, 3), nn.Conv2d(c2, 4 * self.reg_max, 1)) for x in ch)
        self.cv3 = nn.ModuleList(nn.Sequential(Conv(x, c3, 3), Conv(c3, c3, 3), nn.Conv2d(c3, self.nc, 1)) for x in ch)
        self.dfl = DFL(self.reg_max) if self.reg_max > 1 else nn.Identity()

    def forward(self, x):
        shape = x[0].shape
        r4 = 4 * self.reg_max
        y, a_off, strides = None, 0, None
        tta = None if self.training else self.__dict__.get('_tta')
        aug = None if tta is None else tta['aug']
        if tta is not None:
            strides = self._cached('stride_list', [self.stride], lambda: [float(v) for v in self.stride.tolist()])
            y, best, a_off = tta['y'], tta['best'], tta['a_off']
        elif not self.training:
            strides = self._cached('stride_list', [self.stride], lambda: [float(v) for v in self.stride.tolist()])
            a_total = sum(t.shape[2] * t.shape[3] for t in x)
            y = torch.empty(shape[0], 4 + self.nc, a_total, dtype=torch.float32, device=x[0].device)
            best = torch.empty(shape[0], a_total, dtype=torch.int64, device=x[0].device)
        decoded = [False] * self.nl
        offs = [None] * self.nl
        for i in range(self.nl):
            if tta is not None and i not in tta['levels']:
                continue
            offs[i] = a_off
            xi = x[i]
            b, _, h, w = xi.shape
            feat = ops.new_act(b, self.no, h, w, self.cv2[i][0].out_dtype(xi), xi.device)
            pk01 = None if self.training else self._merged_first(i, xi, feat.dtype)
            if pk01 is not None:
                xq = self.q8_site(('first01', i), xi) if feat.dtype == torch.bfloat16 else None
                t01 = ops.conv2d(xi, pk01, 1, ops.ACT_SILU) if xq is None else ops.conv2d_fp8(xi, self._merged_first(i, xi, feat.dtype, xq), 1, ops.ACT_SILU)
                c2 = self.cv2[i][0].conv.out_channels
                tc = self.cv3[i][1](t01[:, c2:])
                box3 = self._box3_in_tail(i, t01[:, :c2], tc, feat.dtype)
                if box3 is not None:
                    pk3, pkb_pad = box3
                    pkc = self._cached((id(self.cv3[i][2]), feat.dtype), [self.cv3[i][2].weight, self.cv3[i][2].bias],
                                       lambda c=self.cv3[i][2]: ops.PackedConv(c.weight, c.bias, None, 1, feat.dtype))
                    ops.detect_tail(t01[:, :c2], tc, pkb_pad, pkc, self.nc, strides[i], a_off, feat, y, best, pk3=pk3, aug=aug)
                    decoded[i] = True
                    a_off += h * w
                    x[i] = feat
                    continue
                tb = self.cv2[i][1](t01[:, :c2])
            else:
                tb = self.cv2[i][1](self.cv2[i][0](xi))
                tc = self.cv3[i][1](self.cv3[i][0](xi))
            if not self.training and ops.detect_tail_supported(tb, tc, self.nc, self.reg_max, feat.dtype):
                pkb = self._cached((id(self.cv2[i][2]), feat.dtype), [self.cv2[i][2].weight, self.cv2[i][2].bias],
                                   lambda c=self.cv2[i][2]: ops.PackedConv(c.weight, c.bias, None, 1, feat.dtype))
                pkc = self._cached((id(self.cv3[i][2]), feat.dtype), [self.cv3[i][2].weight, self.cv3[i][2].bias],
                                   lambda c=self.cv3[i][2]: ops.PackedConv(c.weight, c.bias, None, 1, feat.dtype))
                ops.detect_tail(tb, tc, pkb, pkc, self.nc, strides[i], a_off, feat, y, best, aug=aug)
                decoded[i] = True
            else:
                _HeadConv.run(self, self.cv2[i][2], tb, feat[:, :r4])
                _HeadConv.run(self, self.cv3[i][2], tc, feat[:, r4:])
            if self.training:
                self._save_ctx((tb, tc))
            else:
                a_off += h * w
            x[i] = feat
        if self.training:
            return x
        if tta is not None:
            for i in tta['levels']:
                if not decoded[i]:
                    ops.detect_decode(x[i], self.reg_max, self.nc, strides[i], offs[i], y, aug=aug, best=best)
            return y, x
        if self.dynamic or self.shape != shape:
            from ...yolo.utils.tal import make_anchors
            self.anchors, self.strides = (t.transpose(0, 1) for t in make_anchors(x, strides, 0.5))
            self.shape = shape
        a_off = 0
        for i, f in enumerate(x):
            if not decoded[i]:
                ops.detect_decode(f, self.reg_max, self.nc, strides[i], a_off, y)
            a_off += f.shape[2] * f.shape[3]
        if all(decoded):
            ops.attach_best_keys(y, best)
        return y if self.export else (y, x)

    def _box3_in_tail(self, i, tb_in, tc, dt):
        m3, m1 = self.cv2[i][1], self.cv2[i][2]
        if (self.training or not ops.FUSED_DETECT_BOX3 or dt != torch.bfloat16 or not isinstance(m3, Conv) or not m3.plain_affine() or not isinstance(m3.act, nn.SiLU)
                or m3.conv.kernel_size != (3, 3) or m3.conv.stride != (1, 1) or m3.conv.groups != 1 or m3.conv.in_channels != 16 or m3.conv.out_channels != 16
                or m3._forward_hooks or m3.__dict__.get('_q8') or ops.Q8_CALIB is not None or tb_in.shape[1] != 16
                or not ops.detect_tail_supported(tb_in, tc, self.nc, self.reg_max, dt)):
            return None
        pk3 = m3.packed(dt, direct=False)

        def pad_pack():
            w = m1.weight.detach().float().reshape(m1.out_channels, 16)
            wp = torch.zeros(m1.out_channels, 32, device=w.device)
            wp[:, :16] = w
            return ops.PackedConv(wp[:, ops.acc_order_index(32, w.device)].reshape(m1.out_channels, 32, 1, 1), m1.bias, None, 1, dt)
        return pk3, self._cached((id(m1), dt, 'acc32'), [m1.weight, m1.bias], pad_pack)

    def _merged_first(self, i, xi, dt, xq=None):
        a, b = self.cv2[i][0], self.cv3[i][0]
        ok = all(isinstance(m, Conv) and m.plain_affine() and isinstance(m.act, nn.SiLU) and m.conv.kernel_size == (3, 3) and m.conv.stride == (1, 1)
                 and m.conv.groups == 1 for m in (a, b))
        fused = ok and not hasattr(a, 'bn')
        if (not ok or fused != (not hasattr(b, 'bn')) or (not fused and a.bn.eps != b.bn.eps) or a.conv.out_channels % 8
                or not ops.conv_can_mfma(xi, a.conv.in_channels, a.conv.out_channels + b.conv.out_channels, 3, 1, 1, dt)):
            return None
        tens = [t for m in (a, b) for t in m.affine_tensors()]
        cat = lambda f: torch.cat([f(a).detach().float(), f(b).detach().float()])
        zb = lambda m: m.conv.bias if m.conv.bias is not None else torch.zeros(m.conv.out_channels, device=m.conv.weight.device)
        bn = lambda: None if fused else (cat(lambda m: m.bn.weight), cat(lambda m: m.bn.bias), cat(lambda m: m.bn.running_mean), cat(lambda m: m.bn.running_var), a.bn.eps)
        cb = lambda: cat(zb) if fused else None
        if xq is not None:
            return self._cached(('first01', i, 'fp8', float(xq)), tens, lambda: ops.PackedConvFp8(cat(lambda m: m.conv.weight), cb(), bn(), 3, xq))
        return self._cached(('first01', i, dt), tens, lambda: ops.PackedConv(cat(lambda m: m.conv.weight), cb(), bn(), 3, dt))

    def backward(self, grads):
        r4 = 4 * self.reg_max
        ctx = [self._ctx.pop() for _ in range(self.nl)][::-1]
        out = []
        for i, g in enumerate(grads):
            tb, tc = ctx[i]
            gb = self.cv2[i][0].backward(self.cv2[i][1].backward(_HeadConv.backward(self.cv2[i][2], tb, g[:, :r4])))
            gc = self.cv3[i][0].backward(self.cv3[i][1].backward(_HeadConv.backward(self.cv3[i][2], tc, g[:, r4:])))
            out.append(ops.add(gb, gc, out=gb))
        return out

    def bias_init(self):
        for a, b, s in zip(self.cv2, self.cv3, self.stride):
            a[-1].bias.data[:] = 1.0
            b[-1].bias.data[:self.nc] = math.log(5 / self.nc / (640 / s) ** 2)


SEG_TRAIN_MSG = ('segmentation training is not built: the reference\'s v8SegmentationLoss cannot run in this fork, so there is nothing to pin a '
                 'training path to; Segment / SegmentationModel are inference modules (call .eval())')


class Segment(Detect):

    def __init__(self, nc=80, nm=32, npr=256, ch=()):
        super().__init__(nc, ch)
        self.nm = nm
        self.npr = npr
        self.proto = Proto(ch[0], self.npr, self.nm)
        c4 = max(ch[0] // 4, self.nm)
        self.cv4 = nn.ModuleList(nn.Sequential(Conv(x, c4, 3), Conv(c4, c4, 3), nn.Conv2d(c4, self.nm, 1)) for x in ch)

    def q8_site(self, key, x, x2=None):
        return None

    def forward(self, x):
        if self.training:
            raise NotImplementedError(SEG_TRAIN_MSG)
        p = self.proto(x[0])
        mcs = []
        for i in range(self.nl):
            t = self.cv4[i][1](self.cv4[i][0](x[i]))
            b, _, h, w = t.shape
            m = ops.new_act(b, self.nm, h, w, t.dtype, t.device)
            _HeadConv.run(self, self.cv4[i][2], t, m)
            mcs.append(m)
        export, self.export = self.export, False
        try:
            y, feats = Detect.forward(self, x)
        finally:
            self.export = export
        cat = ops.seg_concat(y, mcs)
        best = ops._best_keys_of(y, y.shape[0], y.shape[2])
        if best is not None:
            ops.attach_best_keys(cat, best)
        mc = cat[:, 4 + self.nc:]
        return (cat, p) if self.export else (cat, (feats, mc, p))

    def backward(self, grads):
        raise NotImplementedError(SEG_TRAIN_MSG)


class Scale(nn.Module):

    def __init__(self, scale=1.0):
        super().__init__()
        self.scale = nn.Parameter(torch.tensor(scale, dtype=torch.float))

    def forward(self, x):
        raise RuntimeError('Scale is a parameter container only: TOODHead.forward never applies it (head.py:537)')


class Conv_GN(HipModule):
    default_act = nn.SiLU()

    def __init__(self, c1, c2, k=1, s=1, p=None, g=1, d=1, act=True):
        super().__init__()
        if d != 1 or g != 1 or (p is not None and p != k // 2):
            raise RuntimeError('Conv_GN: only dense, dilation-1, same-padding convolutions are built')
        self.conv = nn.Conv2d(c1, c2, k, s, k // 2, groups=g, dilation=d, bias=False)
        self.gn = nn.GroupNorm(16, c2)
        self.act = self.default_act if act is True else act if isinstance(act, nn.Module) else nn.Identity()

    def forward(self, x, out=None):
        from .conv import act_code
        dt = self.out_dtype(x)
        k, st = self.conv.kernel_size[0], self.conv.stride[0]
        mfma = ops.conv_can_mfma(x, self.conv.in_channels, self.conv.out_channels, k, st, 1, dt)
        pk = self._cached(('raw', dt, not mfma), [self.conv.weight], lambda: ops.PackedConv(self.conv.weight, None, None, k, dt, direct=not mfma))
        y = ops.conv2d(x, pk, st, ops.ACT_NONE)
        z = ops.groupnorm(y, self.gn.weight.detach().float(), self.gn.bias.detach().float(), self.gn.num_groups, self.gn.eps, act_code(self.act), out=out)
        if self.training:
            self._save_ctx((x, y))
        return z

    def backward(self, g, accumulate=False):
        from .conv import act_code
        x, y = self._ctx.pop()
        for p in (self.conv.weight, self.gn.weight, self.gn.bias):
            ops.grad_buf(p)
        dy = ops.gn_act_bwd(g, y, self.gn.weight.detach().float(), self.gn.bias.detach().float(), self.gn.num_groups, self.gn.eps, act_code(self.act),
                            self.gn.weight.grad, self.gn.bias.grad, accumulate)
        k = self.conv.kernel_size[0]
        ops.conv_wgrad(x, dy, k, 1, self.conv.weight.grad, accumulate=accumulate)
        return ops.conv_dgrad(dy, self.conv.weight, k, 1, ops.like(x))


class _ConvModuleBias(nn.Module):

    def __init__(self, c1, c2):
        super().__init__()
        self.conv = nn.Conv2d(c1, c2, 1, bias=True)
        self.activate = nn.ReLU(inplace=True)


class TaskDecomposition(HipModule):

    def __init__(self, feat_channels, stacked_convs, la_down_rate=8, conv_cfg=None, norm_cfg=None):
        super().__init__()
        if norm_cfg is not None:
            raise RuntimeError('TaskDecomposition: norm_cfg is None everywhere in the reference head')
        self.feat_channels, self.stacked_convs = feat_channels, stacked_convs
        self.in_channels = feat_channels * stacked_convs
        self.la_conv1 = nn.Conv2d(self.in_channels, self.in_channels // la_down_rate, 1)
        self.relu = nn.ReLU(inplace=True)
        self.la_conv2 = nn.Conv2d(self.in_channels // la_down_rate, stacked_convs, 1, padding=0)
        self.sigmoid = nn.Sigmoid()
        self.reduction_conv = _ConvModuleBias(self.in_channels, feat_channels)

    def forward(self, feat, sums=None):
        f32 = lambda t: t.detach().float().reshape(t.shape[0], -1).contiguous()
        la = self._cached('la', [self.la_conv1.weight, self.la_conv1.bias, self.la_conv2.weight, self.la_conv2.bias],
                          lambda: (f32(self.la_conv1.weight), self.la_conv1.bias.detach().float().contiguous(), f32(self.la_conv2.weight),
                                   self.la_conv2.bias.detach().float().contiguous()))
        scale = ops.tood_layer_attn(feat, la[0], la[1], la[2], la[3], self.stacked_convs, sums=sums)
        rc = self.reduction_conv.conv
        dt = self.out_dtype(feat)
        pk = self._cached(('red', dt), [rc.weight], lambda: ops.PackedConv(rc.weight, None, None, 1, dt))
        out = ops.conv2d(feat, pk, 1, ops.ACT_RELU, in_scale=scale)
        if self.training:
            self._save_ctx((feat, scale, sums if sums is not None else ops.nc_reduce(feat), out, la))
        return out

    def backward(self, g, accumulate=False):
        feat, scale, sums, out, la = self._ctx.pop()
        rc = self.reduction_conv.conv
        for p in (rc.weight, self.la_conv1.weight, self.la_conv1.bias, self.la_conv2.weight, self.la_conv2.bias):
            ops.grad_buf(p)
        gr = ops.relu_mask(g, out)
        ops.conv_wgrad(ops.channel_affine(feat, scale, None), gr, 1, 1, rc.weight.grad, accumulate=accumulate)
        t = ops.conv_dgrad(gr, rc.weight, 1, 1, ops.like(feat))
        dscale = ops.nc_reduce(t, feat)
        dsums = ops.tood_layer_attn_bwd(sums, dscale, feat.shape[2] * feat.shape[3], la[0], la[1], la[2], la[3], self.stacked_convs,
                                        self.la_conv1.weight.grad, self.la_conv1.bias.grad, self.la_conv2.weight.grad, self.la_conv2.bias.grad, accumulate)
        return t, scale, dsums


class _DCNParams(nn.Module):

    def __init__(self, c1, c2, bias):
        super().__init__()
        self.weight = nn.Parameter(torch.empty(c2, c1, 3, 3))
        self.bias = nn.Parameter(torch.zeros(c2)) if bias else None
        nn.init.kaiming_uniform_(self.weight, a=5 ** 0.5)


class DyDCNv2(HipModule):

    def __init__(self, in_channels, out_channels, stride=1, norm_cfg=dict(type='GN', num_groups=16, requires_grad=True)):
        super().__init__()
        if stride != 1:
            raise RuntimeError('DyDCNv2: stride 1 only (the head never uses another)')
        self.with_norm = norm_cfg is not None
        self.conv = _DCNParams(in_channels, out_channels, bias=not self.with_norm)
        if self.with_norm:
            self.norm = nn.GroupNorm(norm_cfg.get('num_groups', 16), out_channels)

    def forward(self, x, offset_mask, act=ops.ACT_NONE):
        cw = self.conv.weight
        if self.training:
            if self.conv.bias is not None or not self.with_norm:
                raise NotImplementedError('DyDCNv2 training: only the normalised, bias-free form the head builds')
            dt = x.dtype
            col = ops.dcn_im2col(x, offset_mask)
            pk1 = self._cached(('col1x1', dt), [cw], lambda: ops.PackedConv(cw.detach().reshape(cw.shape[0], cw.shape[1] * 9, 1, 1), None, None, 1, dt))
            d = ops.conv2d(col, pk1, 1, ops.ACT_NONE)
            z = ops.groupnorm(d, self.norm.weight.detach().float(), self.norm.bias.detach().float(), self.norm.num_groups, self.norm.eps, act)
            self._save_ctx((x, offset_mask, col, d, act))
            return z
        wg = self._cached('gemm', [cw], lambda: cw.detach().float().permute(2, 3, 1, 0).reshape(9 * cw.shape[1], cw.shape[0]).contiguous())
        b = None if self.conv.bias is None else self.conv.bias.detach().float()
        if (b is None and x.dtype == torch.bfloat16 and offset_mask.dtype == x.dtype and cw.shape[1] % 8 == 0 and cw.shape[0] % 16 == 0 and cw.shape[0] <= 64
                and ops.is_nhwc(x) and ops.is_nhwc(offset_mask)):
            pk = self._cached('mfma', [cw], lambda: ops.PackedConv(cw, None, None, 3, torch.bfloat16))
            y = ops.dcnv2_mfma(x, offset_mask, pk)
        else:
            y = ops.dcnv2(x, offset_mask, wg, b, cw.shape[0])
        if not self.with_norm:
            return y
        return ops.groupnorm(y, self.norm.weight.detach().float(), self.norm.bias.detach().float(), self.norm.num_groups, self.norm.eps, act, out=y)


    def backward(self, g, accumulate=False):
        x, om, col, d, act = self._ctx.pop()
        cw = self.conv.weight
        for p in (cw, self.norm.weight, self.norm.bias):
            ops.grad_buf(p)
        gd = ops.gn_act_bwd(g, d, self.norm.weight.detach().float(), self.norm.bias.detach().float(), self.norm.num_groups, self.norm.eps, act,
                            self.norm.weight.grad, self.norm.bias.grad, accumulate)
        w1 = cw.detach().reshape(cw.shape[0], cw.shape[1] * 9, 1, 1)
        ops.conv_wgrad(col, gd, 1, 1, cw.grad.view(cw.shape[0], cw.shape[1] * 9, 1, 1), accumulate=accumulate)
        gcol = ops.conv_dgrad(gd, w1, 1, 1, ops.like(col))
        return ops.dcn_col2im_bwd(gcol, x, om)


class TOODHead(Detect):

    def __init__(self, nc, hidc, ch=()):
        HipModule.__init__(self)
        self.nc = nc
        self.nl = len(ch)
        self.reg_max = 16
        self.no = nc + self.reg_max * 4
        self.stride = torch.zeros(self.nl)
        if any(c != hidc for c in ch):
            raise RuntimeError(f'TOODHead: every input level must have hidc={hidc} channels, got {list(ch)} (the reference YAML passes hidc unscaled, '
                               'tasks.py:664-665)')
        self.share_conv = nn.Sequential(Conv_GN(hidc, hidc // 2, 3), Conv_GN(hidc // 2, hidc // 2, 3))
        self.cls_decomp = TaskDecomposition(hidc // 2, 2, 16)
        self.reg_decomp = TaskDecomposition(hidc // 2, 2, 16)
        self.DyDCNV2 = DyDCNv2(hidc // 2, hidc // 2)
        self.spatial_conv_offset = nn.Conv2d(hidc, 3 * 3 * 3, 3, padding=1)
        self.offset_dim = 2 * 3 * 3
# ... 117 lines not shown
```

mgdt_yolo_amd/ops.py:

```python
import ctypes as C
import os

import torch

from . import _lib as L
from ._lib import ACT_GELU, ACT_NONE, ACT_RELU, ACT_SILU, BF16, F32, View

U8 = 2
_DT = {torch.float32: F32, torch.bfloat16: BF16}


def dtype_code(dt):
    try:
        return _DT[dt]
    except KeyError:
        raise RuntimeError(f'mgdt_yolo_amd computes in float32 or bfloat16, not {dt}') from None


def _need_gpu(t):
    if not t.is_cuda:
        raise RuntimeError('mgdt_yolo_amd runs on MI355X (HIP) only: got a CPU tensor and there is no CPU/PyTorch fallback')


_PROF = None


def _launch(name, symbol, *args, meta=None):
    fn = getattr(L.lib(), symbol)
    if _PROF is None:
        L.check(fn(*args), name)
        return
    e0, e1 = torch.cuda.Event(enable_timing=True), torch.cuda.Event(enable_timing=True)
    e0.record()
    L.check(fn(*args), name)
    e1.record()
    _PROF.append((name, meta or _META.pop(name, None), e0, e1))


_META = {}


class profile:

    def __enter__(self):
        global _PROF
        _PROF = self._raw = []
        return self

    def __exit__(self, *exc):
        global _PROF
        _PROF = None
        torch.cuda.synchronize()
        self.rows = [(n, m, a.elapsed_time(b)) for n, m, a, b in self._raw]
        return False


def stream():
    return C.c_void_p(torch.cuda.current_stream().cuda_stream)


SIDE_STREAM = os.environ.get('MGDT_SIDE_STREAM', '1') != '0'
_SIDE = {}


def side_stream(device):
    dev = torch.device(device).index if torch.device(device).index is not None else torch.cuda.current_device()
    key = (dev, _LANE[0])
    if key not in _SIDE:
        _SIDE[key] = torch.cuda.Stream(device=dev)
    return _SIDE[key]


_FORCE_CTX = [0]


def ctx_enabled():
    return _FORCE_CTX[0] > 0 or torch.is_grad_enabled()


class force_ctx:
    def __enter__(self):
        _FORCE_CTX[0] += 1

    def __exit__(self, *exc):
        _FORCE_CTX[0] -= 1
        return False


def view(t):
    _need_gpu(t)
    b, c, h, w = t.shape
    sn, sc, sh, sw = t.stride()
    return View(t.data_ptr(), b, h, w, c, sn, sh, sw, sc)


def vp(t):
    return C.byref(view(t)) if t is not None else None


def ptr(t):
    if t is None:
        return None
    _need_gpu(t)
    return C.c_void_p(t.data_ptr())


def _same(*ts):
    ts = [t for t in ts if t is not None]
    for t in ts[1:]:
        if t.dtype != ts[0].dtype:
            raise RuntimeError(f'mgdt_yolo_amd: operands of one kernel must share a dtype, got {[str(u.dtype) for u in ts]}')


def new_act(b, c, h, w, dtype, device):
    return torch.empty((b, c, h, w), dtype=dtype, device=device, memory_format=torch.channels_last)


def is_nhwc(t):
    return t.stride(1) == 1


def grad_buf(p):
    if p.grad is None:
        p.grad = torch.zeros_like(p)
    return p.grad


def like(t):
    return new_act(t.shape[0], t.shape[1], t.shape[2], t.shape[3], t.dtype, t.device)


class PackedConv:
    __slots__ = ('w', 'bias', 'k', 'cin', 'cout', 'dtype', 'direct', 'groups', 'src', 'epoch', '__weakref__')

    def __init__(self, weight, conv_bias, bn, k, dtype, direct=False, groups=1):
        lib = L.lib()
        weight = weight.detach().float().contiguous()
        _need_gpu(weight)
        cout, cin_g = weight.shape[0], weight.shape[1]
        dev = weight.device
        g, b, mu, var, eps = (None, None, None, None, 0.0) if bn is None else bn
        f = lambda t: None if t is None else t.detach().float().contiguous()
        g, b, mu, var, cb = f(g), f(b), f(mu), f(var), f(conv_bias)
        self.k, self.cin, self.cout, self.dtype, self.direct, self.groups = k, cin_g * groups, cout, dtype, direct, groups
        if direct:
            self.w = torch.empty(k * k * cin_g * cout, dtype=torch.float32, device=dev)
            self.bias = torch.empty(cout, dtype=torch.float32, device=dev)
            _launch('conv_pack_direct', 'mgdt_conv_pack_direct', ptr(weight), ptr(cb), ptr(g), ptr(b), ptr(mu), ptr(var), eps, cin_g, cout, k,
                                              ptr(self.w), ptr(self.bias), stream())
        else:
            code = dtype_code(dtype)
            nbytes = lib.mgdt_conv_packed_bytes(cin_g, cout, k, code)
            self.w = torch.empty(nbytes, dtype=torch.uint8, device=dev)
            self.bias = torch.empty((cout + 15) // 16 * 16, dtype=torch.float32, device=dev)
            _launch('conv_pack', 'mgdt_conv_pack', ptr(weight), ptr(cb), ptr(g), ptr(b), ptr(mu), ptr(var), eps, cin_g, cout, k, code,
                                       ptr(self.w), ptr(self.bias), stream())
            if groups == 1:
                _register_pack(self, (weight, cb, g, b, mu, var, float(eps), cin_g, cout, k, code, 0))


class PackedConvFp8:
    __slots__ = ('w', 'bias', 'oscale', 'xq', 'k', 'cin', 'cout', 'dtype', 'direct', 'groups', '__weakref__')

    def __init__(self, weight, conv_bias, bn, k, xq):
        lib = L.lib()
        weight = weight.detach().float().contiguous()
        _need_gpu(weight)
        cout, cin = weight.shape[0], weight.shape[1]
        dev = weight.device
        g, b, mu, var, eps = (None, None, None, None, 0.0) if bn is None else bn
        f = lambda t: None if t is None else t.detach().float().contiguous()
        g, b, mu, var, cb = f(g), f(b), f(mu), f(var), f(conv_bias)
        self.k, self.cin, self.cout, self.dtype, self.direct, self.groups, self.xq = k, cin, cout, torch.bfloat16, False, 1, float(xq)
        self.w = torch.empty(lib.mgdt_conv_packed_bytes_fp8(cin, cout, k), dtype=torch.uint8, device=dev)
        cpad = (cout + 15) // 16 * 16
        self.bias = torch.empty(cpad, dtype=torch.float32, device=dev)
        self.oscale = torch.empty(cpad, dtype=torch.float32, device=dev)
        _launch('conv_pack_fp8', 'mgdt_conv_pack_fp8', ptr(weight), ptr(cb), ptr(g), ptr(b), ptr(mu), ptr(var), eps, cin, cout, k, self.xq,
                ptr(self.w), ptr(self.bias), ptr(self.oscale), stream())


Q8_CALIB = None
Q8_CALIB_PCT = None


def conv2d_fp8(x, pk, stride, act, out=None, x2=None, r1=None, r2=None, in_scale=None, in_shift=None):
    _need_gpu(x)
    b, _, h, w = x.shape
    ho, wo = conv_out_hw(h, w, pk.k, stride)
    if out is None:
        out = new_act(b, pk.cout, ho, wo, torch.bfloat16, x.device)
    _same(x, x2, r1, r2, out)
    if x.dtype != torch.bfloat16:
        raise RuntimeError(f'conv2d_fp8: activations are bf16 in HBM, the input is {x.dtype}')
    if _PROF is not None:
        _META['conv2d_fp8_fwd'] = dict(shape=(b, pk.cin, h, w, pk.cout, pk.k, stride), flops=2.0 * b * ho * wo * pk.cout * pk.cin * pk.k * pk.k,
                                       bytes=float(b * h * w * pk.cin * 2 + b * ho * wo * pk.cout * 2 + pk.cout * pk.cin * pk.k * pk.k))
    _launch('conv2d_fp8_fwd', 'mgdt_conv2d_fp8_fwd', vp(x), vp(x2), ptr(in_scale), ptr(in_shift), ptr(pk.w), ptr(pk.bias), ptr(pk.oscale), pk.xq,
            pk.k, stride, act, vp(r1), vp(r2), vp(out), stream())
    return out


_PACK_REGISTRY = None
LIVE_STORAGES = set()


def _register_pack(obj, src):
    global _PACK_REGISTRY
    import weakref
    if not all(t is None or t.untyped_storage().data_ptr() in LIVE_STORAGES for t in src[:6]):
        return
    if _PACK_REGISTRY is None:
        _PACK_REGISTRY = weakref.WeakSet()
    obj.src, obj.epoch = src, PARAM_EPOCH[0]
    _PACK_REGISTRY.add(obj)


def repack_all():
    if not _PACK_REGISTRY:
        return []
    live = [o for o in _PACK_REGISTRY if getattr(o, 'epoch', -2) == PARAM_EPOCH[0] - 1]
    if not live:
        return []
    arr = (L.PackDesc * len(live))()
    for d, o in zip(arr, live):
        w, cb, g, b, mu, var, eps, cin, cout, k, code, mode = o.src
        d.w, d.conv_bias, d.bn_gamma, d.bn_beta, d.bn_mean, d.bn_var = ptr(w), ptr(cb), ptr(g), ptr(b), ptr(mu), ptr(var)
        d.bn_eps, d.cin, d.cout, d.k, d.dtype, d.mode = eps, cin, cout, k, code, mode
        d.packed, d.bias_out = ptr(o.w), ptr(o.bias)
    _launch('conv_pack_batch', 'mgdt_conv_pack_batch', arr, len(live), stream())
    for o in live:
        o.epoch = PARAM_EPOCH[0]
    return live


def pack_is_current(obj):
    return getattr(obj, 'epoch', None) == PARAM_EPOCH[0]


def conv_can_mfma(x, cin, cout, k, s, groups, dtype):
    pe = 8 if dtype == torch.bfloat16 else 4
    return (groups == 1 and k in (1, 3) and s in (1, 2) and cin % pe == 0 and cout % 4 == 0 and x.dtype == dtype
            and is_nhwc(x) and x.stride(3) % pe == 0 and x.stride(2) % pe == 0 and x.stride(0) % pe == 0
            and x.data_ptr() % 16 == 0)


def conv_out_hw(h, w, k, s):
    p = k // 2
    return (h + 2 * p - k) // s + 1, (w + 2 * p - k) // s + 1


def conv2d(x, pk, stride, act, out=None, x2=None, r1=None, r2=None, in_scale=None, in_shift=None):
    _need_gpu(x)
    b, _, h, w = x.shape
    ho, wo = conv_out_hw(h, w, pk.k, stride)
    if out is None:
        out = new_act(b, pk.cout, ho, wo, pk.dtype, x.device)
    if _PROF is not None:
        es = out.element_size()
        _META['conv2d_direct_fwd' if pk.direct else 'conv2d_fwd'] = dict(
            shape=(b, pk.cin, h, w, pk.cout, pk.k, stride), flops=2.0 * b * ho * wo * pk.cout * pk.cin // pk.groups * pk.k * pk.k,
            bytes=float(b * h * w * pk.cin * x.element_size() + b * ho * wo * pk.cout * es + pk.w.numel() * pk.w.element_size()))
    if pk.direct:
        if x2 is not None or r1 is not None or r2 is not None or in_scale is not None or in_shift is not None:
            raise RuntimeError('direct convolution path has no fused extras')
        _launch('conv2d_direct_fwd', 'mgdt_conv2d_direct_fwd', vp(x), U8 if x.dtype == torch.uint8 else dtype_code(x.dtype), ptr(pk.w), ptr(pk.bias), pk.k, stride, pk.groups, act,
                                           vp(out), dtype_code(out.dtype), stream())
    else:
        _same(x, x2, r1, r2, out)
        if x.dtype != pk.dtype:
            raise RuntimeError(f'conv2d: the weights are packed for {pk.dtype}, the input is {x.dtype}')
        _launch('conv2d_fwd', 'mgdt_conv2d_fwd', vp(x), vp(x2), ptr(in_scale), ptr(in_shift), ptr(pk.w), ptr(pk.bias), pk.k, stride, act,
                                    vp(r1), vp(r2), vp(out), dtype_code(pk.dtype), stream())
    return out


def spr_attention(x, fc1_w, fc1_b, fc2_w, fc2_b, groups, softmax=True):
    b, c, h, w = x.shape
    lib = L.lib()
    part = torch.empty(b * L.SPR_SPLITS * c * 5, dtype=torch.float32, device=x.device)
    _launch('spr_pool_fwd', 'mgdt_spr_pool_fwd', vp(x), ptr(part), dtype_code(x.dtype), stream())
    attn = torch.empty(b, c, dtype=torch.float32, device=x.device)
    _launch('spr_attn_fwd', 'mgdt_spr_attn_fwd', ptr(part), ptr(fc1_w), ptr(fc1_b), ptr(fc2_w), ptr(fc2_b), b, c, groups, h, w, int(bool(softmax)),
            ptr(attn), stream())
    return attn


def spr_attention_scale(x, fc1_w, fc1_b, fc2_w, fc2_b, groups, out=None, part=None, nsplit=0, tiles=(0, 0), pools=()):
    b, c, h, w = x.shape
    if part is None:
        part = torch.empty(b * L.SPR_SPLITS * c * 5, dtype=torch.float32, device=x.device)
        _launch('spr_pool_fwd', 'mgdt_spr_pool_fwd', vp(x), ptr(part), dtype_code(x.dtype), stream())
        nsplit, tiles = L.SPR_SPLITS, (0, 0)
    out = like(x) if out is None else out
    pools = list(pools)
    if len(pools) > 2:
        raise RuntimeError('spr_attention_scale: at most two pooled outputs')
    _same(x, out, *pools)
    pa, pb = (pools + [None, None])[:2]
    _launch('spr_attn_scale_fwd', 'mgdt_spr_attn_scale_fwd', ptr(part), int(nsplit), int(tiles[0]), int(tiles[1]), ptr(fc1_w), ptr(fc1_b), ptr(fc2_w), ptr(fc2_b), groups, vp(x), vp(out),
            vp(pa), vp(pb), dtype_code(x.dtype), stream())
    return out


FUSED_NECK = True


FUSED_STEM = True


class PackedStem2:

    def __init__(self, weight, bn):
        g, b, mu, var, eps = bn
        scale = (g.detach().float() / torch.sqrt(eps + var.detach().float()))
        wf = (weight.detach().float() * scale.view(-1, 1, 1, 1)).contiguous()
        self.bias = (b.detach().float() - g.detach().float() * mu.detach().float() / torch.sqrt(var.detach().float() + eps)).contiguous()
        self.blob = torch.empty(L.lib().mgdt_stem2_packed_bytes(), dtype=torch.uint8, device=weight.device)
        L.check(L.lib().mgdt_stem2_pack(ptr(wf), ptr(self.blob), stream()), 'stem2_pack')


def stem2(x, pk0, pk1):
    _need_gpu(x)
    b, _, h, w = x.shape
    h0, w0 = (h - 1) // 2 + 1, (w - 1) // 2 + 1
    h1, w1 = (h0 - 1) // 2 + 1, (w0 - 1) // 2 + 1
    y = new_act(b, 32, h1, w1, torch.bfloat16, x.device)
    if _PROF is not None:
        _META['stem2_fwd'] = dict(shape=(b, 3, h, w, 32, 3, 4), flops=2.0 * b * (h0 * w0 * 16 * 27 + h1 * w1 * 32 * 144),
                                  bytes=float(x.numel() * x.element_size() + y.numel() * 2))
    _launch('stem2_fwd', 'mgdt_stem2_fwd', vp(x), U8 if x.dtype == torch.uint8 else dtype_code(x.dtype), ptr(pk0.blob), ptr(pk0.bias), ptr(pk1.w), ptr(pk1.bias),
            vp(y), stream())
    return y


FUSED_CSP_BLOCK = True
CSP_MSPA, CSP_C2F = 0, 1


def csp_block_supported(mode, x, cout, wd, nbtl, dtype):
    if not (FUSED_CSP_BLOCK and dtype == torch.bfloat16 and x.dtype == dtype and is_nhwc(x)):
        return False
    lib = L.lib()
    if not lib.mgdt_csp_block_supported(mode, x.shape[1], int(cout), int(wd), int(nbtl), x.shape[2], x.shape[3], dtype_code(dtype)):
        return False
    return lib.mgdt_csp_block_tiles(mode, x.shape[0], x.shape[1], int(cout), int(wd), int(nbtl), x.shape[2], x.shape[3], None) > 0


def csp_block(mode, x, front, front_bias, mids, shortcut, back, wd, act, cout, want_pool):
    lib = L.lib()
    b, cin, h, w = x.shape
    nb = len(mids) // 2
    geom = (C.c_int * 8)()
    slots = lib.mgdt_csp_block_tiles(mode, b, cin, cout, wd, nb, h, w, geom)
    if slots <= 0:
        raise RuntimeError('csp_block: configuration not covered')
    y = new_act(b, cout, h, w, x.dtype, x.device)
    pool = torch.empty(b * slots * cout, dtype=torch.float32, device=x.device) if want_pool else None
    marr = (C.c_void_p * len(mids))(*[m.w.data_ptr() for m in mids])
    barr = (C.c_void_p * len(mids))(*[m.bias.data_ptr() for m in mids])
    if _PROF is not None:
        es = x.element_size()
        catc = (3 if mode == CSP_MSPA else 2) * wd + nb * wd
        fl = 2.0 * b * h * w * ((3 * wd * wd if mode == CSP_MSPA else 0) + 2 * nb * 9 * wd * wd + catc * cout)
        _META['csp_block_fwd'] = dict(shape=(b, cin, h, w, cout, wd, nb), flops=fl, bytes=float(b * h * w * (cin + cout) * es))
    _launch('csp_block_fwd', 'mgdt_csp_block_fwd', mode, vp(x), ptr(front), ptr(front_bias), marr, barr, nb, int(bool(shortcut)), ptr(back.w), ptr(back.bias),
            int(wd), act, vp(y), ptr(pool), dtype_code(x.dtype), stream())
    return y, pool, slots, (geom[6], geom[7])


def scale_channels(x, attn, out=None):
    out = like(x) if out is None else out
    _same(x, out)
    _launch('scale_channels_fwd', 'mgdt_scale_channels_fwd', vp(x), ptr(attn), vp(out), dtype_code(x.dtype), stream())
    return out


def sppf_pools(x, y1, y2, y3):
    _launch('sppf_pool_fwd', 'mgdt_sppf_pool_fwd', vp(x), vp(y1), vp(y2), vp(y3), dtype_code(x.dtype), stream())


def adaptive_avgpool(x, out):
    _same(x, out)
    _launch('adaptive_avgpool_fwd', 'mgdt_adaptive_avgpool_fwd', vp(x), vp(out), dtype_code(x.dtype), stream())
    return out


def bilinear(x, out):
    _same(x, out)
    _launch('bilinear_fwd', 'mgdt_bilinear_fwd', vp(x), vp(out), dtype_code(x.dtype), stream())
    return out


def nearest(x, out):
    _same(x, out)
    _launch('nearest_fwd', 'mgdt_nearest_fwd', vp(x), vp(out), dtype_code(x.dtype), stream())
    return out


def copy(x, out):
    _launch('copy_fwd', 'mgdt_copy_fwd', vp(x), U8 if x.dtype == torch.uint8 else dtype_code(x.dtype), vp(out), dtype_code(out.dtype), stream())
    return out


def dwconv7_ln(x, dw_w49c, dw_b, ln_w, ln_b, eps, out=None):
    out = like(x) if out is None else out
    _launch('dwconv7_ln_fwd', 'mgdt_dwconv7_ln_fwd', vp(x), ptr(dw_w49c), ptr(dw_b), ptr(ln_w), ptr(ln_b), eps, vp(out), dtype_code(x.dtype),
                                        stream())
    return out


def grn_scale(t, gamma):
    b, c = t.shape[:2]
    ws = torch.empty(b * L.GRN_SPLITS * c, dtype=torch.float32, device=t.device)
    sc = torch.empty(b, c, dtype=torch.float32, device=t.device)
    _launch('grn_stats_fwd', 'mgdt_grn_stats_fwd', vp(t), ptr(gamma), ptr(ws), ptr(sc), dtype_code(t.dtype), stream())
    return sc


FUSED_PW_CHAIN = True


def pw_chain_supported(wd, dtype):
    return FUSED_PW_CHAIN and L.lib().mgdt_pw_chain_packed_bytes(int(wd), dtype_code(dtype)) > 0


class PackedPwChain:

    def __init__(self, convs, dtype):
        wd = convs[0][0].shape[0]
        self.wd, self.dtype = wd, dtype
        self.blob = torch.empty(L.lib().mgdt_pw_chain_packed_bytes(wd, dtype_code(dtype)), dtype=torch.uint8, device=convs[0][0].device)
        f = lambda t: None if t is None else t.detach().float().contiguous()
        for i, (w, cb, bn) in enumerate(convs):
            g, b, mu, var, eps = (None, None, None, None, 0.0) if bn is None else bn
            w, cb, g, b, mu, var = f(w), f(cb), f(g), f(b), f(mu), f(var)
            L.check(L.lib().mgdt_pw_chain_pack(i, ptr(w), ptr(cb), ptr(g), ptr(b), ptr(mu), ptr(var), eps, wd, dtype_code(dtype), ptr(self.blob), stream()),
                    'pw_chain_pack')


def pw_chain3(x, pk, act, out):
    if _PROF is not None:
        b, c, h, w = x.shape
        _META['pw_chain3_fwd'] = dict(shape=(b, pk.wd, h, w, pk.wd, 1, 1), flops=2.0 * b * h * w * pk.wd * pk.wd * 3, bytes=float(2 * b * h * w * c * x.element_size()))
    _launch('pw_chain3_fwd', 'mgdt_pw_chain3_fwd', vp(x), ptr(pk.blob), pk.wd, act, vp(out), dtype_code(x.dtype), stream())
    return out


FUSED_CNX_MLP = True


def cnx_mlp_supported(c, dtype):
    return FUSED_CNX_MLP and L.lib().mgdt_cnx_mlp_packed_bytes(int(c), dtype_code(dtype)) > 0


class PackedCnxMlp:

    def __init__(self, w1, b1, w2, b2, dtype):
        c = w2.shape[0]
        dev = w1.device
        self.c, self.dtype = c, dtype
        self.blob = torch.empty(L.lib().mgdt_cnx_mlp_packed_bytes(c, dtype_code(dtype)), dtype=torch.uint8, device=dev)
        f = lambda t: t.detach().float().contiguous()
        w1, b1, w2, b2 = f(w1), f(b1), f(w2), f(b2)
        L.check(L.lib().mgdt_cnx_mlp_pack(ptr(w1), ptr(b1), ptr(w2), ptr(b2), c, ptr(self.blob), dtype_code(dtype), stream()))


def cnx_mlp(t, res, pk, gamma, beta, out=None):
    b, c, h, w = t.shape
    out = like(t) if out is None else out
    ws = torch.empty(L.lib().mgdt_cnx_mlp_workspace_bytes(b, h, w, c), dtype=torch.uint8, device=t.device)
    if _PROF is not None:
        _META['cnx_mlp_fwd'] = dict(shape=(b, c, h, w, c, 1, 1), flops=2.0 * b * h * w * c * 4 * c * 3, bytes=float(4 * b * h * w * c * t.element_size()))
    _launch('cnx_mlp_fwd', 'mgdt_cnx_mlp_fwd', vp(t), vp(res), ptr(pk.blob), ptr(gamma), ptr(beta), ptr(ws), vp(out), dtype_code(t.dtype), stream())
    return out


FUSED_CNX_BLOCK = True
FUSED_CNX_TAIL = True
_CNX_WS = {}
_LANE = [0]


class lane:

    def __init__(self, i):
        self.i = int(i)

    def __enter__(self):
        self.prev, _LANE[0] = _LANE[0], self.i

    def __exit__(self, *exc):
        _LANE[0] = self.prev
        return False


def cnx_block_supported(x, dtype):
    b, c, h, w = x.shape
    return bool(FUSED_CNX_BLOCK and x.dtype == dtype and is_nhwc(x) and L.lib().mgdt_cnx_block_supported(b, h, w, c, dtype_code(dtype)))


def cnx_block(x, dw_w49c, dw_b, ln_w, ln_b, eps, pk, gamma, beta, out=None, tail=None, tail_act=0):
    b, c, h, w = x.shape
    if out is None:
        out = like(x) if tail is None else new_act(b, tail.cout, h, w, x.dtype, x.device)
    if out.data_ptr() == x.data_ptr():
        raise RuntimeError('cnx_block: the output may not alias the input (tiles read their neighbours\' halo)')
    nbytes = L.lib().mgdt_cnx_block_workspace_bytes(b, h, w, c)
    key = (x.device, b, c, h, w, _LANE[0])
    ws = _CNX_WS.get(key)
    if ws is None:
        if torch.cuda.is_current_stream_capturing():
            raise RuntimeError('cnx_block: run the model once before capturing it into a graph (the kernel\'s barrier words are allocated and zeroed on first use)')
        ws = _CNX_WS[key] = torch.zeros(nbytes, dtype=torch.uint8, device=x.device)
    if _PROF is not None:
        _META['cnx_block_fwd'] = dict(shape=(b, c, h, w, c, 7, 1), flops=2.0 * b * h * w * c * (4 * c * 2 + 49), bytes=float(2 * b * h * w * c * x.element_size()))
    _launch('cnx_block_fwd', 'mgdt_cnx_block_fwd', vp(x), ptr(dw_w49c), ptr(dw_b), ptr(ln_w), ptr(ln_b), float(eps), ptr(pk.blob), ptr(gamma), ptr(beta),
            None if tail is None else ptr(tail.w), None if tail is None else ptr(tail.bias), int(tail_act), ptr(ws), nbytes, vp(out), dtype_code(x.dtype), stream())
    return out


FUSED_INJECT = True


def conv1x1_inject_supported(x, cout, ga, dtype):
    return bool(FUSED_INJECT and x.dtype == dtype and ga.dtype == dtype and is_nhwc(x) and is_nhwc(ga) and
                L.lib().mgdt_conv1x1_inject_supported(x.shape[1], cout, x.shape[2], x.shape[3], ga.shape[2], ga.shape[3], dtype_code(dtype)))


def acc_order_index(c, device):
    k = torch.arange(c, device=device)
    j, g, e = k // 32, (k // 8) % 4, k % 8
    return (2 * j + e // 4) * 16 + 4 * g + e % 4


def conv1x1_inject_conv_supported(x, cmid, cout2, ga, dtype):
    return bool(FUSED_INJECT and FUSED_INJECT_CONV and x.dtype == dtype and ga.dtype == dtype and is_nhwc(x) and is_nhwc(ga) and
                L.lib().mgdt_conv1x1_inject_conv_supported(x.shape[1], cmid, cout2, x.shape[2], x.shape[3], ga.shape[2], ga.shape[3], dtype_code(dtype)))


def conv1x1_inject_conv(x, pk, ga, gf, pk2, act2, out, gsrc=None, pkg=None):
    b, _, h, w = x.shape
    _same(x, ga, gf, gsrc, out)
    if _PROF is not None:
        _META['conv1x1_inject_conv_fwd'] = dict(shape=(b, pk.cin, h, w, pk2.cout, 1, 1), flops=2.0 * b * h * w * (pk.cout * pk.cin + pk2.cout * pk2.cin),
                                                bytes=float(b * h * w * (pk.cin + pk2.cout) * x.element_size() + (2 * ga.numel() * ga.element_size() if gsrc is None else gsrc.numel() * 2)))
    _launch('conv1x1_inject_conv_fwd', 'mgdt_conv1x1_inject_conv_fwd', vp(x), ptr(pk.w), ptr(pk.bias), vp(ga), vp(gf), vp(gsrc), None if pkg is None else ptr(pkg.w),
            None if pkg is None else ptr(pkg.bias), pk.cout, ptr(pk2.w), ptr(pk2.bias), int(act2), vp(out), dtype_code(pk.dtype), stream())
    return out


FUSED_INJECT_CONV = True
FUSED_INJECT_GCONV = True


def conv1x1_inject(x, pk, ga, gf, out=None):
    b, _, h, w = x.shape
    if out is None:
        out = new_act(b, pk.cout, h, w, pk.dtype, x.device)
    if _PROF is not None:
        _META['conv1x1_inject_fwd'] = dict(shape=(b, pk.cin, h, w, pk.cout, 1, 1), flops=2.0 * b * h * w * pk.cout * pk.cin,
                                           bytes=float(b * h * w * (pk.cin + pk.cout) * x.element_size() + 2 * ga.numel() * ga.element_size()))
    _launch('conv1x1_inject_fwd', 'mgdt_conv1x1_inject_fwd', vp(x), ptr(pk.w), ptr(pk.bias), vp(ga), vp(gf), vp(out), dtype_code(pk.dtype), stream())
    return out


def groupnorm(x, gamma, beta, groups, eps, act, out=None):
    b, c = x.shape[:2]
    out = like(x) if out is None else out
    ws = torch.empty(L.lib().mgdt_groupnorm_workspace_bytes(b, c), dtype=torch.uint8, device=x.device)
    _launch('groupnorm_fwd', 'mgdt_groupnorm_fwd', vp(x), ptr(gamma), ptr(beta), groups, float(eps), act, ptr(ws), vp(out), dtype_code(x.dtype), stream())
    return out


def tood_layer_attn(feat, w1, b1, w2, b2, stacked, sums=None):
    b, c, h, w = feat.shape
    sums = nc_reduce(feat) if sums is None else sums
# ... 727 lines not shown
```

Measured before the change: 40540 images/sec.

## Split merged head conv output into two dense tensors; write detect-tail rows as lines

The merged first conv of the detect head (box and class branches) now writes its two channel ranges into separate contiguous NHWC tensors from the LDS 3x3 kernel. Downstream convs and the detect tail therefore read dense inputs instead of strided slices of a concatenated tensor. The detect tail also gains a LINES variant that buffers 32 anchors per wave and flushes full 128-byte output rows with vector stores instead of 16-anchor fragments. Debug SKIP template variants are added, and the kernel now launches through hipLaunchKernel with per-variant attribute setup.

New measurement: 40830 images/sec, median of 6. Within noise of the previous version (+0.7%).

```diff
diff --git a/include/mgdt.h b/include/mgdt.h
--- a/include/mgdt.h
+++ b/include/mgdt.h
@@ -38,6 +38,9 @@
 int mgdt_conv2d_fwd(const mgdt_view* x, const mgdt_view* x2, const float* in_scale, const float* in_shift,
                     const void* packed_w, const float* bias, int k, int stride, int act, const mgdt_view* r1,
                     const mgdt_view* r2, const mgdt_view* y, int dtype, mgdt_stream s);
+int mgdt_conv2d_split_supported(const mgdt_view* x, int k, int stride, int act, const mgdt_view* y_lo, const mgdt_view* y_hi, int dtype);
+int mgdt_conv2d_split_fwd(const mgdt_view* x, const void* packed_w, const float* bias, int k, int stride, int act, const mgdt_view* y_lo,
+                          const mgdt_view* y_hi, int dtype, mgdt_stream s);
 size_t mgdt_conv_packed_bytes_fp8(int cin, int cout, int k);
 int mgdt_conv_pack_fp8(const float* w_oihw, const float* conv_bias, const float* bn_gamma, const float* bn_beta, const float* bn_mean,
                        const float* bn_var, float bn_eps, int cin, int cout, int k, float x_qscale, void* packed_out, float* bias_out,
diff --git a/mgdt_yolo_amd/_lib.py b/mgdt_yolo_amd/_lib.py
--- a/mgdt_yolo_amd/_lib.py
+++ b/mgdt_yolo_amd/_lib.py
@@ -34,6 +34,8 @@
     'mgdt_conv_packed_bytes': (_sz, [_i, _i, _i, _i]),
     'mgdt_conv_pack': (_i, [_vp, _vp, _vp, _vp, _vp, _vp, _f, _i, _i, _i, _i, _vp, _vp, _vp]),
     'mgdt_conv2d_fwd': (_i, [VP, VP, _vp, _vp, _vp, _vp, _i, _i, _i, VP, VP, VP, _i, _vp]),
+    'mgdt_conv2d_split_supported': (_i, [VP, _i, _i, _i, VP, VP, _i]),
+    'mgdt_conv2d_split_fwd': (_i, [VP, _vp, _vp, _i, _i, _i, VP, VP, _i, _vp]),
     'mgdt_conv_packed_bytes_fp8': (_sz, [_i, _i, _i]),
     'mgdt_conv_pack_fp8': (_i, [_vp, _vp, _vp, _vp, _vp, _vp, _f, _i, _i, _i, _f, _vp, _vp, _vp, _vp]),
     'mgdt_conv2d_fp8_fwd': (_i, [VP, VP, _vp, _vp, _vp, _vp, _vp, _f, _i, _i, _i, VP, VP, VP, _vp]),
diff --git a/mgdt_yolo_amd/csrc/conv3x3_lds.hip b/mgdt_yolo_amd/csrc/conv3x3_lds.hip
--- a/mgdt_yolo_amd/csrc/conv3x3_lds.hip
+++ b/mgdt_yolo_amd/csrc/conv3x3_lds.hip
@@ -11,6 +11,7 @@
 struct C3Args {
   const char* x; int xsn, xsh, xsw; uint32_t x_bytes;
   char* y; int ysn, ysh, ysw; uint32_t y_bytes;
+  char* y2; int y2sn, y2sh, y2sw; uint32_t y2_bytes; int c_split;
   const char* wpk; const float* bias;
   int N, H, W, Ho, Wo, Cin, Cout, CP, nchunks, NTtot, ncg, tiles_x, tiles_per_img, ntiles, XP, act;
   FastDiv fd_tpi, fd_tx, fd_cp;
@@ -41,6 +42,7 @@
   const int nb0 = cg * NBW;
   const __amdgpu_buffer_rsrc_t xrs = __builtin_amdgcn_make_buffer_rsrc((void*)a.x, 0, a.x_bytes, 0x00020000);
   const __amdgpu_buffer_rsrc_t yrs = __builtin_amdgcn_make_buffer_rsrc((void*)a.y, 0, a.y_bytes, 0x00020000);
+  const __amdgpu_buffer_rsrc_t yrs2 = __builtin_amdgcn_make_buffer_rsrc((void*)a.y2, 0, a.c_split ? a.y2_bytes : 0u, 0x00020000);
 
   for (int p = tid; p < a.nchunks * 4; p += NTHR) {
     const int tap = (int)fdiv((uint32_t)p, a.fd_cp), cp = p - tap * a.CP;
@@ -173,15 +175,16 @@
       for (int m = 0; m < MT; ++m) {
         const int oy = tyi * TH + wave * MT + m, ox = txi * C3_TW + r;
         const bool pin = oy < a.Ho && ox < a.Wo;
-        const int po = n * a.ysn + oy * a.ysh + ox * a.ysw;
+        const int po = n * a.ysn + oy * a.ysh + ox * a.ysw, po2 = n * a.y2sn + oy * a.y2sh + ox * a.y2sw;
 #pragma unroll
         for (int bw = 0; bw < NBH; ++bw) {
           const int co = (nbw0 + bw) * 16 + 4 * g;
+          const bool hi = a.c_split && (nbw0 + bw) * 16 >= a.c_split;
           bf16x4 o;
 #pragma unroll
           for (int j = 0; j < 4; ++j) o[j] = (bf16)c3_act<ACT>(Q8 ? acc[bw][m][j] * osc[Q8 ? bw : 0][j] : acc[bw][m][j]);
-          __builtin_amdgcn_raw_buffer_store_b64(__builtin_bit_cast(__attribute__((__vector_size__(2 * sizeof(unsigned int)))) unsigned int, o), yrs,
-                                                (pin && co < a.Cout) ? (uint32_t)(po + co * 2) : (uint32_t)C3_OOB, 0, 0);
+          __builtin_amdgcn_raw_buffer_store_b64(__builtin_bit_cast(__attribute__((__vector_size__(2 * sizeof(unsigned int)))) unsigned int, o), hi ? yrs2 : yrs,
+                                                (pin && co < a.Cout) ? (uint32_t)(hi ? po2 + (co - a.c_split) * 2 : po + co * 2) : (uint32_t)C3_OOB, 0, 0);
         }
       }
     }
@@ -192,24 +195,27 @@
 }
 
 bool mgdt_conv3x3_lds_launch(const mgdt_view* x, const mgdt_view* y, const void* packed_w, const float* bias, int act, int CP, int nchunks, int NTtot, hipStream_t st,
-                             const float* q8_oscale, float q8_xq, int stride) {
+                             const float* q8_oscale, float q8_xq, int stride, const mgdt_view* y2, bool dry_run) {
   const bool q8 = q8_oscale != nullptr;
   static const int mode = getenv("MGDT_CONV3_LDS") ? atoi(getenv("MGDT_CONV3_LDS")) : 1;
   if (!mode) return false;
   static const bool ws2 = !(getenv("MGDT_C3_WAVES8") && atoi(getenv("MGDT_C3_WAVES8")) == 0);
   const bool wide = mode >= 3 || ws2;
-  const int Cin = x->c, Cout = y->c;
+  const int Cin = x->c, Cout = y->c + (y2 ? y2->c : 0);
+  if (y2 && (q8 || stride != 1 || y->c % 16 || y->c <= 0 || y2->c <= 0)) return false;
   if (stride == 2 && (q8_oscale || Cin > 64 || NTtot % 4 || (nchunks != 9 && !(nchunks == 18 && wide)))) return false;
   if (Cin % 8 || Cin < 32 || Cin > 80 || Cout % 4 || Cout < 32 || (act != MGDT_ACT_SILU && act != MGDT_ACT_NONE && act != MGDT_ACT_RELU)) return false;
   const long M = (long)x->n * x->h * x->w;
   if (M < 16 * 1024 || x->h < 16 || x->w < 16) return false;
   const long extx = ((long)(x->n - 1) * x->sn + (long)(x->h - 1) * x->sh + (long)(x->w - 1) * x->sw + x->c) * 2;
   const long exty = ((long)(y->n - 1) * y->sn + (long)(y->h - 1) * y->sh + (long)(y->w - 1) * y->sw + y->c) * 2;
-  if (extx >= 0x7fffffffL || exty >= 0x7fffffffL) return false;
+  const long exty2 = y2 ? ((long)(y2->n - 1) * y2->sn + (long)(y2->h - 1) * y2->sh + (long)(y2->w - 1) * y2->sw + y2->c) * 2 : 0;
+  if (extx >= 0x7fffffffL || exty >= 0x7fffffffL || exty2 >= 0x7fffffffL) return false;
   C3Args a;
   memset(&a, 0, sizeof(a));
   a.x = (const char*)x->p; a.xsn = (int)(x->sn * 2); a.xsh = (int)(x->sh * 2); a.xsw = (int)(x->sw * 2); a.x_bytes = (uint32_t)extx;
   a.y = (char*)y->p; a.ysn = (int)(y->sn * 2); a.ysh = (int)(y->sh * 2); a.ysw = (int)(y->sw * 2); a.y_bytes = (uint32_t)exty;
+  if (y2) { a.y2 = (char*)y2->p; a.y2sn = (int)(y2->sn * 2); a.y2sh = (int)(y2->sh * 2); a.y2sw = (int)(y2->sw * 2); a.y2_bytes = (uint32_t)exty2; a.c_split = y->c; }
   a.wpk = (const char*)packed_w; a.bias = bias;
   a.N = x->n; a.H = x->h; a.W = x->w; a.Ho = y->h; a.Wo = y->w; a.Cin = Cin; a.Cout = Cout; a.CP = CP; a.nchunks = nchunks; a.NTtot = NTtot; a.act = act;
   a.XP = q8 ? Cin + 16 : Cin * 2 + 16;
@@ -235,6 +241,7 @@
   nwg = (int)std::min<long>(nwg, (long)a.ntiles * a.ncg);
   nwg = nwg / a.ncg * a.ncg;
   if (nwg < a.ncg) return false;
+  if (dry_run) return true;
  #define C3_LAUNCH_Q8(NB, ACTV)                                                                                      \
   {                                                                                                                  \
     static std::atomic<bool> qattr{false}, qattr18{false}, qattr23{false};                                            \
diff --git a/mgdt_yolo_amd/csrc/conv_igemm.hip b/mgdt_yolo_amd/csrc/conv_igemm.hip
--- a/mgdt_yolo_amd/csrc/conv_igemm.hip
+++ b/mgdt_yolo_amd/csrc/conv_igemm.hip
@@ -306,7 +306,7 @@
 }
 
 bool mgdt_conv3x3_lds_launch(const mgdt_view* x, const mgdt_view* y, const void* packed_w, const float* bias, int act, int CP, int nchunks, int NTtot, hipStream_t st,
-                             const float* q8_oscale, float q8_xq, int stride);
+                             const float* q8_oscale, float q8_xq, int stride, const mgdt_view* y2 = nullptr, bool dry_run = false);
 
 template <typename T, int NT, int MT, bool Q8>
 int launch_igemm(const ConvArgs& a, int gx, int gy, int threads, size_t lds, hipStream_t st);
@@ -336,6 +336,29 @@
                                const void* packed_w, const float* bias, int k, int stride, int act, const mgdt_view* r1,
                                const mgdt_view* r2, const mgdt_view* y, int dtype, mgdt_stream s) {
   return conv2d_fwd_impl(x, x2, in_scale, in_shift, packed_w, bias, k, stride, act, r1, r2, y, dtype, 0, s);
+}
+static int conv2d_split_impl(const mgdt_view* x, const void* packed_w, const float* bias, int k, int stride, int act, const mgdt_view* y_lo, const mgdt_view* y_hi,
+                             int dtype, mgdt_stream s, bool dry_run) {
+  if (!view_ok(x) || !view_ok(y_lo) || !view_ok(y_hi) || (!dry_run && (!packed_w || !bias))) MGDT_FAIL(MGDT_BAD_ARG, "conv2d_split: null/empty view or weights");
+  if (dtype != MGDT_BF16 || k != 3 || stride != 1) MGDT_FAIL(MGDT_BAD_SHAPE, "conv2d_split: built for bf16 3x3 stride 1 (dtype %d k %d stride %d)", dtype, k, stride);
+  for (const mgdt_view* y : {y_lo, y_hi})
+    if (y->n != x->n || y->h != x->h || y->w != x->w) MGDT_FAIL(MGDT_BAD_SHAPE, "conv2d_split: y is %dx%dx%d, expected %dx%dx%d", y->n, y->h, y->w, x->n, x->h, x->w);
+  if (x->c % 8 || y_lo->c % 16 || y_hi->c % 4) MGDT_FAIL(MGDT_BAD_SHAPE, "conv2d_split: cin=%d %% 8, c_lo=%d %% 16, c_hi=%d %% 4 must be 0", x->c, y_lo->c, y_hi->c);
+  auto aligned = [&](const mgdt_view* v, int q) { return v->sc == 1 && v->sw % q == 0 && v->sh % q == 0 && v->sn % q == 0 && ((uintptr_t)v->p % (q * 2)) == 0; };
+  if (!aligned(x, 8) || !aligned(y_lo, 4) || !aligned(y_hi, 4)) MGDT_FAIL(MGDT_BAD_SHAPE, "conv2d_split: x/y must be NHWC views (sc==1) with 16-byte aligned pieces");
+  int CP, nchunks, NTtot;
+  conv_geometry(x->c, y_lo->c + y_hi->c, 3, dtype, &CP, &nchunks, &NTtot, 0);
+  if (!mgdt_conv3x3_lds_launch(x, y_lo, packed_w, bias, act, CP, nchunks, NTtot, (hipStream_t)s, nullptr, 1.f, 1, y_hi, dry_run))
+    MGDT_FAIL(MGDT_BAD_SHAPE, "conv2d_split: %dx%dx%d cin %d cout %d+%d is not covered by the LDS-staged 3x3 kernel", x->n, x->h, x->w, x->c, y_lo->c, y_hi->c);
+  if (!dry_run) MGDT_CHECK_LAUNCH("conv2d_split(3x3 lds)");
+  return MGDT_OK;
+}
+extern "C" int mgdt_conv2d_split_fwd(const mgdt_view* x, const void* packed_w, const float* bias, int k, int stride, int act, const mgdt_view* y_lo,
+                                     const mgdt_view* y_hi, int dtype, mgdt_stream s) {
+  return conv2d_split_impl(x, packed_w, bias, k, stride, act, y_lo, y_hi, dtype, s, false);
+}
+extern "C" int mgdt_conv2d_split_supported(const mgdt_view* x, int k, int stride, int act, const mgdt_view* y_lo, const mgdt_view* y_hi, int dtype) {
+  return conv2d_split_impl(x, nullptr, nullptr, k, stride, act, y_lo, y_hi, dtype, nullptr, true) == MGDT_OK;
 }
 extern "C" int mgdt_conv2d_phase_fwd(const mgdt_view* x, const void* packed_w, const float* bias, int phase, const mgdt_view* r1, const mgdt_view* r2,
                                      const mgdt_view* y, int dtype, mgdt_stream s) {
diff --git a/mgdt_yolo_amd/csrc/detect_tail.hip b/mgdt_yolo_amd/csrc/detect_tail.hip
--- a/mgdt_yolo_amd/csrc/detect_tail.hip
+++ b/mgdt_yolo_amd/csrc/detect_tail.hip
@@ -18,7 +18,10 @@
 constexpr int DT_THREADS = 256;
 constexpr int DT_P = 20;
 constexpr int DT_WT = (2 * 16 + 4) * DT_P;
-
+constexpr int DT_PL = 36;
+static_assert((16 + 4) * DT_PL <= DT_WT, "the 32-anchor tiles live in the same per-wave LDS as the 16-anchor ones");
+
+template <bool LINES, int SKIP>
 __global__ __launch_bounds__(DT_THREADS) void detect_tail_kernel(const DtArgs a) {
   extern __shared__ __attribute__((aligned(16))) char smem[];
   char* wbl = smem;
@@ -55,7 +58,7 @@
   };
   auto flush = [&](const float* tile, int nrow, int row0, int n, int an0) __attribute__((always_inline)) {
     const int row = lane >> 2, q = (lane & 3) * 4;
-    if (row < nrow && row0 + row < 4 + a.nc) {
+    if (!(SKIP & 1) && row < nrow && row0 + row < 4 + a.nc) {
       float* dst = a.y + ((size_t)n * (4 + a.nc) + row0 + row) * a.a_total + a.a_off + an0 + q;
       const float* src = tile + row * DT_P + q;
       if (vec_ok) { if (an0 + q < a.HW) *(f32x4*)dst = *(const f32x4*)src; }
@@ -63,6 +66,15 @@
 #pragma unroll
         for (int e = 0; e < 4; ++e) if (an0 + q + e < a.HW) dst[e] = src[e];
       }
+    }
+  };
+  auto flush_line = [&](const float* tile, int nrow, int row0, int n, int a0) __attribute__((always_inline)) {
+    const int q = (lane & 7) * 4;
+#pragma unroll
+    for (int pass = 0; pass < 2; ++pass) {
+      const int row = pass * 8 + (lane >> 3);
+      if (!(SKIP & 1) && row < nrow && row0 + row < 4 + a.nc && a0 + q < a.HW)
+        *(f32x4*)(a.y + ((size_t)n * (4 + a.nc) + row0 + row) * a.a_total + a.a_off + a0 + q) = *(const f32x4*)(tile + row * DT_PL + q);
     }
   };
   int flip = 0;
@@ -70,6 +82,8 @@
     const int n = unit / a.units_per_img, a0 = (unit - n * a.units_per_img) * 32;
     float bs[2] = {-1.f, -1.f};
     int bcl[2] = {0, 0};
+    bf16x8 BcL[LINES ? 2 : 1][4];
+    int foL[2] = {MGDT_OOB, MGDT_OOB};
 #pragma unroll
     for (int u = 0; u < 2; ++u) {
       const int an = a0 + u * 16 + r;
@@ -86,7 +100,7 @@
           const int p = kc * 4 + g, tap = p >> 1, cp = p & 1;
           const int iy = oy + tap / 3 - 1, ix = ox + tap % 3 - 1;
           const bool ok = pv && tap < 9 && (unsigned)iy < (unsigned)a.H && (unsigned)ix < (unsigned)a.W;
-          B3[kc] = __builtin_bit_cast(bf16x8, __builtin_amdgcn_raw_buffer_load_b128(brs, ok ? (uint32_t)(n * a.bsn + iy * a.bsh + ix * a.bsw + cp * 16) : (uint32_t)MGDT_OOB, 0, 0));
+          B3[kc] = __builtin_bit_cast(bf16x8, __builtin_amdgcn_raw_buffer_load_b128(brs, (ok && !(SKIP & 4)) ? (uint32_t)(n * a.bsn + iy * a.bsh + ix * a.bsw + cp * 16) : (uint32_t)MGDT_OOB, 0, 0));
         }
         f32x4 acc3 = *(const f32x4*)(bias3l + 4 * g);
 #pragma unroll
@@ -108,7 +122,7 @@
       float lb[4];
 #pragma unroll
       for (int j = 0; j < 4; ++j) lb[j] = (float)(bf16)accb[j];
-      bstore4<bf16>(frs, (uint32_t)fo + (uint32_t)(4 * g * 2), f32x4{lb[0], lb[1], lb[2], lb[3]});
+      if (!(SKIP & 2)) bstore4<bf16>(frs, (uint32_t)fo + (uint32_t)(4 * g * 2), f32x4{lb[0], lb[1], lb[2], lb[3]});
       const float mx = fmaxf(fmaxf(lb[0], lb[1]), fmaxf(lb[2], lb[3]));
       float den = 0.f, num = 0.f;
 #pragma unroll
@@ -126,6 +140,13 @@
         comp = comp / a.aug_s;
         if (g == 0 && a.aug_flip) comp = a.aug_w - comp;
       }
+      if constexpr (LINES) {
+        yt[(16 + g) * DT_PL + u * 16 + r] = comp;
+#pragma unroll
+        for (int kc = 0; kc < 4; ++kc) BcL[u][kc] = Bc[kc];
+        foL[u] = fo;
+        continue;
+      }
       {
         float* bt = yt + 32 * DT_P;
         bt[g * DT_P + r] = comp;
@@ -141,7 +162,7 @@
         float lc[4];
 #pragma unroll
         for (int j = 0; j < 4; ++j) lc[j] = (float)(bf16)acc[j];
-        bstore4<bf16>(frs, c < a.nc ? (uint32_t)fo + (uint32_t)((r4 + c) * 2) : (uint32_t)MGDT_OOB, f32x4{lc[0], lc[1], lc[2], lc[3]});
+        if (!(SKIP & 2)) bstore4<bf16>(frs, c < a.nc ? (uint32_t)fo + (uint32_t)((r4 + c) * 2) : (uint32_t)MGDT_OOB, f32x4{lc[0], lc[1], lc[2], lc[3]});
         float* ct = yt + flip * 16 * DT_P;
         flip ^= 1;
 #pragma unroll
@@ -152,6 +173,33 @@
         }
         wave_sync();
         flush(ct, 16, 4 + nb * 16, n, a0 + u * 16);
+      }
+    }
+    if constexpr (LINES) {
+      wave_sync();
+      flush_line(yt + 16 * DT_PL, 4, 0, n, a0);
+      for (int nb = 0; nb < a.nbc; ++nb) {
+        const int c = nb * 16 + 4 * g;
+        wave_sync();
+#pragma unroll
+        for (int u = 0; u < 2; ++u) {
+          f32x4 acc = *(const f32x4*)(biasl + 16 + nb * 16 + 4 * g);
+#pragma unroll
+          for (int kc = 0; kc < 4; ++kc)
+            if (kc < a.kch) acc = mma(*(const bf16x8*)(wlane_c + (size_t)(kc * a.nbc + nb) * 1024), BcL[u][kc], acc);
+          float lc[4];
+#pragma unroll
+          for (int j = 0; j < 4; ++j) lc[j] = (float)(bf16)acc[j];
+          if (!(SKIP & 2)) bstore4<bf16>(frs, c < a.nc ? (uint32_t)foL[u] + (uint32_t)((r4 + c) * 2) : (uint32_t)MGDT_OOB, f32x4{lc[0], lc[1], lc[2], lc[3]});
+#pragma unroll
+          for (int j = 0; j < 4; ++j) {
+            const float sg = fast_sigmoid(lc[j]);
+            yt[(4 * g + j) * DT_PL + u * 16 + r] = sg;
+            if (c + j < a.nc && sg > bs[u]) { bs[u] = sg; bcl[u] = c + j; }
+          }
+        }
+        wave_sync();
+        flush_line(yt, 16, 4 + nb * 16, n, a0);
       }
     }
     if (a.best) {
@@ -209,14 +257,25 @@
   a.aug = aug ? 1 : 0; a.aug_flip = aug_flip ? 1 : 0; a.aug_s = aug_scale; a.aug_w = aug_img_w;
   const size_t lds = 1024 + (size_t)a.kch * a.nbc * 1024 + (size_t)(16 + a.nbc * 16) * 4 + (size_t)4 * DT_WT * 4 + 5 * 1024 + 64;
   if (lds > 150 * 1024) MGDT_FAIL(MGDT_BAD_SHAPE, "detect_tail: nc=%d needs %zu B of LDS", nc, lds);
-  static size_t attr = 0;
-  if (lds > 64 * 1024 && lds > attr) {
-    hipError_t e = hipFuncSetAttribute((const void*)detect_tail_kernel, hipFuncAttributeMaxDynamicSharedMemorySize, 150 * 1024);
+  static const bool lines_on = !(getenv("MGDT_DT_LINES") && atoi(getenv("MGDT_DT_LINES")) == 0);
+  const bool lines = lines_on && a.HW % 4 == 0 && a_off % 32 == 0 && a_total % 32 == 0 && (uintptr_t)y % 128 == 0;
+  static const int skip = getenv("MGDT_DT_SKIP") ? atoi(getenv("MGDT_DT_SKIP")) : 0;
+  const void* kfn = nullptr;
+#define DT_PICK(L, S) if (lines == L && skip == S) kfn = (const void*)detect_tail_kernel<L, S>;
+  DT_PICK(true, 0) DT_PICK(false, 0) DT_PICK(true, 1) DT_PICK(false, 1) DT_PICK(true, 2) DT_PICK(false, 2) DT_PICK(true, 4) DT_PICK(false, 4)
+#undef DT_PICK
+  if (!kfn) MGDT_FAIL(MGDT_BAD_ARG, "detect_tail: MGDT_DT_SKIP=%d is not instantiated (1, 2 or 4)", skip);
+  static bool attr[8] = {};
+  const int ki = (lines ? 4 : 0) + (skip == 4 ? 3 : skip);
+  if (lds > 64 * 1024 && !attr[ki]) {
+    hipError_t e = hipFuncSetAttribute(kfn, hipFuncAttributeMaxDynamicSharedMemorySize, 150 * 1024);
     if (e != hipSuccess) MGDT_FAIL(MGDT_LAUNCH_FAIL, "detect_tail: hipFuncSetAttribute: %s", hipGetErrorString(e));
-    attr = 150 * 1024;
+    attr[ki] = true;
   }
   const int grid = std::min(cdiv(a.units, 4), 1024);
-  detect_tail_kernel<<<grid, DT_THREADS, lds, (hipStream_t)s>>>(a);
+  void* kargs[] = {(void*)&a};
+  hipError_t le = hipLaunchKernel(kfn, dim3(grid), dim3(DT_THREADS), kargs, lds, (hipStream_t)s);
+  if (le != hipSuccess) MGDT_FAIL(MGDT_LAUNCH_FAIL, "detect_tail: launch: %s", hipGetErrorString(le));
   MGDT_CHECK_LAUNCH("detect_tail_fwd");
   return MGDT_OK;
 }
diff --git a/mgdt_yolo_amd/nn/modules/head.py b/mgdt_yolo_amd/nn/modules/head.py
--- a/mgdt_yolo_amd/nn/modules/head.py
+++ b/mgdt_yolo_amd/nn/modules/head.py
@@ -76,20 +76,24 @@
             pk01 = None if self.training else self._merged_first(i, xi, feat.dtype)
             if pk01 is not None:
                 xq = self.q8_site(('first01', i), xi) if feat.dtype == torch.bfloat16 else None
-                t01 = ops.conv2d(xi, pk01, 1, ops.ACT_SILU) if xq is None else ops.conv2d_fp8(xi, self._merged_first(i, xi, feat.dtype, xq), 1, ops.ACT_SILU)
                 c2 = self.cv2[i][0].conv.out_channels
-                tc = self.cv3[i][1](t01[:, c2:])
-                box3 = self._box3_in_tail(i, t01[:, :c2], tc, feat.dtype)
+                if xq is None and tta is None and type(self) is Detect and ops.conv2d_split_supported(xi, pk01, 1, ops.ACT_SILU, c2):
+                    t0, t1 = ops.conv2d_split(xi, pk01, 1, ops.ACT_SILU, c2)
+                else:
+                    t01 = ops.conv2d(xi, pk01, 1, ops.ACT_SILU) if xq is None else ops.conv2d_fp8(xi, self._merged_first(i, xi, feat.dtype, xq), 1, ops.ACT_SILU)
+                    t0, t1 = t01[:, :c2], t01[:, c2:]
+                tc = self.cv3[i][1](t1)
+                box3 = self._box3_in_tail(i, t0, tc, feat.dtype)
                 if box3 is not None:
                     pk3, pkb_pad = box3
                     pkc = self._cached((id(self.cv3[i][2]), feat.dtype), [self.cv3[i][2].weight, self.cv3[i][2].bias],
                                        lambda c=self.cv3[i][2]: ops.PackedConv(c.weight, c.bias, None, 1, feat.dtype))
-                    ops.detect_tail(t01[:, :c2], tc, pkb_pad, pkc, self.nc, strides[i], a_off, feat, y, best, pk3=pk3, aug=aug)
+                    ops.detect_tail(t0, tc, pkb_pad, pkc, self.nc, strides[i], a_off, feat, y, best, pk3=pk3, aug=aug)
                     decoded[i] = True
                     a_off += h * w
                     x[i] = feat
                     continue
-                tb = self.cv2[i][1](t01[:, :c2])
+                tb = self.cv2[i][1](t0)
             else:
                 tb = self.cv2[i][1](self.cv2[i][0](xi))
                 tc = self.cv3[i][1](self.cv3[i][0](xi))
diff --git a/mgdt_yolo_amd/ops.py b/mgdt_yolo_amd/ops.py
--- a/mgdt_yolo_amd/ops.py
+++ b/mgdt_yolo_amd/ops.py
@@ -273,6 +273,28 @@
         _launch('conv2d_fwd', 'mgdt_conv2d_fwd', vp(x), vp(x2), ptr(in_scale), ptr(in_shift), ptr(pk.w), ptr(pk.bias), pk.k, stride, act,
                                     vp(r1), vp(r2), vp(out), dtype_code(pk.dtype), stream())
     return out
+
+
+SPLIT_FIRST_CONV = True
+
+
+def conv2d_split_supported(x, pk, stride, act, c_lo):
+    if not SPLIT_FIRST_CONV or pk.direct or pk.dtype != torch.bfloat16 or x.dtype != pk.dtype or not x.is_cuda or not 0 < c_lo < pk.cout:
+        return False
+    b, _, h, w = x.shape
+    mk = lambda c: L.View(16, b, h, w, c, h * w * c, w * c, c, 1)
+    return bool(L.lib().mgdt_conv2d_split_supported(vp(x), pk.k, stride, act, C.byref(mk(c_lo)), C.byref(mk(pk.cout - c_lo)), dtype_code(pk.dtype)))
+
+
+def conv2d_split(x, pk, stride, act, c_lo):
+    _need_gpu(x)
+    b, _, h, w = x.shape
+    lo, hi = new_act(b, c_lo, h, w, pk.dtype, x.device), new_act(b, pk.cout - c_lo, h, w, pk.dtype, x.device)
+    if _PROF is not None:
+        _META['conv2d_fwd'] = dict(shape=(b, pk.cin, h, w, pk.cout, pk.k, stride), flops=2.0 * b * h * w * pk.cout * pk.cin * pk.k * pk.k,
+                                   bytes=float(b * h * w * pk.cin * 2 + b * h * w * pk.cout * 2 + pk.w.numel() * pk.w.element_size()))
+    _launch('conv2d_fwd', 'mgdt_conv2d_split_fwd', vp(x), ptr(pk.w), ptr(pk.bias), pk.k, stride, act, vp(lo), vp(hi), dtype_code(pk.dtype), stream())
+    return lo, hi
 
 
 def spr_attention(x, fc1_w, fc1_b, fc2_w, fc2_b, groups, softmax=True):
```
